# cwi-dis/cwipc_util

Hardware: AMD Instinct MI355X
Metric: Mpoints/s filtered (voxel downsample, 10M-pt synthetic) + achieved HBM GB/s (higher is better)
Workload: dtype f32 coordinates in, i64 fixed-point sums, u8 colours; 1 GPU; cwipc_synthetic(10000000) -> cwipc_downsample(+0.01) [BASELINE configs[1]]; points_per_gpu=9998244, bytes_per_gpu=159971904, outputs_per_gpu=39548, fused_points=39548, input_copies_rotated=4, inputs_resident_in_hbm=True

## Files before the change

### cwipc_util_amd/csrc/kernels_voxel.hip

```cpp
#include "internal.hpp"

#include <atomic>
#include <chrono>

#include <cstring>
#include <rocprim/device/device_radix_sort.hpp>

#include <cfloat>
#include <type_traits>
#include <cmath>

#include "voxel_anchor.hpp"
#include "voxel_common.hpp"

namespace cwipc_amd {

namespace {

#include "voxel_k1_general.inc"
#include "voxel_k1_fast.inc"
#include "voxel_partition.inc"
#include "voxel_finalize.inc"

struct PendingVoxel : DeferredResult {
    std::recursive_mutex lock;
    std::shared_ptr<DeviceSoA> src, spec_dst, result;
    volatile unsigned long long *words = nullptr;
    hipStream_t stream = nullptr;
    uint32_t seq = 0, spec_cap = 0;
    float cellsize = 0;
    bool known = false, ok = false, settled = false;
    uint32_t err = 0, m = 0;
    bool leaf_split = true;
    GridSpec gspec{0, 0u, 0u, 0ull};
    bool partitioned = false;
    uint32_t scatter = 0, steps_total = 0;
    uint32_t leaves = 0;
    bool outcome_locked();
    bool outcome() { std::lock_guard<std::recursive_mutex> g(lock); return outcome_locked(); }
    std::shared_ptr<DeviceSoA> settle() override;
};

std::atomic<size_t> g_workspace_bytes{0};
constexpr size_t GRID_BYTES = (size_t)CELLS * RECORD_WORDS * 8;
constexpr size_t HEAD_CTRL_BYTES = 256;

struct Workspace {
    int device = -1;
    size_t grid_bytes = 0;
    int cus = 0, cus_device = -1;
    uint32_t leaf_cap = 0;
    size_t list_cap = 0;
    size_t bbox_cap = 0;
    void *head = nullptr;
    size_t head_bytes = 0;
    int parity = 0;
    uint32_t seq = 0;
    uint32_t last_m = 0;
    uint32_t last_m_grid = 0;
    int shrink = 0;
    int calm = 0;
    bool incoherent = false;
    bool no_fast = false;
    int streak = 0;
    int roomy = 0;
    uint32_t shrink_to = 0;
    void note_leaves(uint32_t leaves) {
        uint32_t need = 4;
        while (need < leaves) need <<= 1;
        if (need * 4 <= leaf_cap) {
            if (++roomy >= 8) shrink_to = need;
        } else {
            roomy = 0;
            shrink_to = 0;
        }
    }
    uint32_t *host_words = nullptr;
    std::shared_ptr<struct PendingVoxel> pending;
    size_t hint_n = 0;
    float hint_cell = 0.f;
    bool hint_split = true;
    bool head_clean[2] = {false, false};
    unsigned long long *leaf_keys = nullptr;
    unsigned long long *hash_keys = nullptr;
    uint32_t *hash_ids = nullptr;
    unsigned long long *records = nullptr;
    uint32_t *occupied = nullptr;
    uint32_t *order = nullptr;
    uint32_t *gbits = nullptr;
    uint32_t *gprefix = nullptr, *gblock = nullptr;
    size_t gwords_cap = 0;
    float *bboxes = nullptr;
    float *part = nullptr;
    size_t part_stride = 0;
    uint32_t *part_hist = nullptr;
    size_t part_rows = 0;
    uint32_t *ctrl = nullptr;
    uint32_t *bitmaps = nullptr;
    uint32_t *seg_count = nullptr;
    float *faces = nullptr;
    uint32_t faces_host[FACE_TABLE_WORDS];
    double faces_mn0[3] = {0, 0, 0};
    double faces_res = 0;
    bool faces_valid = false;
    void drop_partition_buffers() {
        if (part) { (void)hipFree(part); g_workspace_bytes -= 16 * part_stride; }
        if (part_hist) (void)hipFree(part_hist);
        part = nullptr; part_hist = nullptr; part_stride = 0; part_rows = 0;
    }
    VoxWork work() const { return VoxWork{leaf_keys, records, occupied, ctrl, bboxes, faces, bitmaps, seg_count, hash_keys, hash_ids}; }
    char *bind_head(int blk) {
        char *h = (char *)head + (size_t)blk * head_bytes;
        ctrl = (uint32_t *)h;
        leaf_keys = (unsigned long long *)(h + HEAD_CTRL_BYTES);
        seg_count = (uint32_t *)(h + HEAD_CTRL_BYTES + (size_t)leaf_cap * 8);
        hash_keys = (unsigned long long *)(h + HEAD_CTRL_BYTES + (size_t)leaf_cap * 8 + (size_t)leaf_cap * RANK_SEGS * sizeof(uint32_t));
        hash_ids = (uint32_t *)((char *)hash_keys + (size_t)leaf_cap * 4 * 8);
        return h;
    }
    void free_grids() {
        if (head) (void)hipFree(head);
        if (records) (void)hipFree(records);
        if (bitmaps) (void)hipFree(bitmaps);
        head = nullptr; ctrl = nullptr; leaf_keys = nullptr; seg_count = nullptr; records = nullptr; bitmaps = nullptr;
        g_workspace_bytes -= grid_bytes;
        grid_bytes = 0;
        leaf_cap = 0;
    }
    void free_index_bitmap() {
        if (gbits) (void)hipFree(gbits);
        if (gprefix) (void)hipFree(gprefix);
        if (gblock) (void)hipFree(gblock);
        gbits = gprefix = gblock = nullptr; gwords_cap = 0;
    }
    void release() {
        free_grids();
        head_bytes = 0;
        if (occupied) (void)hipFree(occupied);
        if (order) (void)hipFree(order);
        free_index_bitmap();
        if (bboxes) (void)hipFree(bboxes);
        drop_partition_buffers();
        if (faces) (void)hipFree(faces);
        if (host_words) (void)hipHostFree(host_words);
        host_words = nullptr;
        occupied = nullptr; order = nullptr; bboxes = nullptr; faces = nullptr;
        list_cap = 0; bbox_cap = 0;
        faces_valid = false;
    }
    ~Workspace() { release(); }
};

std::mutex g_ws_pool_mutex;
std::vector<Workspace *> *g_ws_pool = new std::vector<Workspace *>();

constexpr int MAX_WS = 2 + ThreadCtx::EXTRA_STREAMS;
struct WorkspaceLease {
    Workspace *ws[MAX_WS] = {nullptr, nullptr, nullptr, nullptr};
    Workspace &get(int which) {
        if (!ws[which]) {
            const int dev = current_device();
            std::lock_guard<std::mutex> lock(g_ws_pool_mutex);
            for (size_t i = 0; i < g_ws_pool->size(); i++) {
                if ((*g_ws_pool)[i]->device == dev) {
                    ws[which] = (*g_ws_pool)[i];
                    g_ws_pool->erase(g_ws_pool->begin() + (long)i);
                    break;
                }
            }
            if (!ws[which]) ws[which] = new Workspace();
        }
        return *ws[which];
    }
    ~WorkspaceLease() {
        bool any = false;
        for (int i = 0; i < MAX_WS; i++) any = any || ws[i];
        if (any) (void)hipDeviceSynchronize();
        for (int i = 0; i < MAX_WS; i++)
            if (ws[i] && ws[i]->pending) (void)ws[i]->pending->outcome();
        std::vector<Workspace *> surplus;
        {
            std::lock_guard<std::mutex> lock(g_ws_pool_mutex);
            for (int i = 0; i < MAX_WS; i++) {
                if (!ws[i]) continue;
                if (g_ws_pool->size() < 8) g_ws_pool->push_back(ws[i]);
                else surplus.push_back(ws[i]);
            }
        }
        for (Workspace *w : surplus) delete w;
    }
};
thread_local WorkspaceLease t_ws;
thread_local int t_ws_next = 0;
thread_local uint32_t t_busy_sample = 0;
thread_local bool t_busy_sampled = false;
thread_local int t_ws_idle = 0;

hipStream_t &workspace_stream(ThreadCtx &c, int i) {
    if (i >= 2) (void)c.extra_stream(i - 2);
    return i == 0 ? c.stream : i == 1 ? c.stream_alt : c.stream_extra[i - 2];
}

struct StreamOfWorkspace {
    ThreadCtx &c;
    hipStream_t *other = nullptr;
    StreamOfWorkspace(ThreadCtx &ctx, int which) : c(ctx) {
        if (which > 0 && workspace_stream(c, which)) other = &workspace_stream(c, which);
        if (other) std::swap(c.stream, *other);
    }
    ~StreamOfWorkspace() {
        if (other) std::swap(c.stream, *other);
    }
};

bool ensure_workspace(Workspace &ws, size_t n, uint32_t leaf_cap, uint32_t nranges, hipStream_t s) {
    const int dev = current_device();
    if (ws.device != dev) {
        ws.release();
        const int lds = (int)sizeof(LdsTable);
        CW_HIP_TRY(hipFuncSetAttribute(reinterpret_cast<const void *>(&voxel_accumulate_kernel<0>), hipFuncAttributeMaxDynamicSharedMemorySize, lds));
        CW_HIP_TRY(hipFuncSetAttribute(reinterpret_cast<const void *>(&voxel_accumulate_kernel<1>), hipFuncAttributeMaxDynamicSharedMemorySize, lds));
        CW_HIP_TRY(hipFuncSetAttribute(reinterpret_cast<const void *>(&voxel_accumulate_kernel<2>), hipFuncAttributeMaxDynamicSharedMemorySize, lds));
        const int lds_fast = (int)sizeof(FastTable);
        CW_HIP_TRY(hipFuncSetAttribute(reinterpret_cast<const void *>(&voxel_accumulate_fast_kernel<0>), hipFuncAttributeMaxDynamicSharedMemorySize, lds_fast));
        CW_HIP_TRY(hipFuncSetAttribute(reinterpret_cast<const void *>(&voxel_accumulate_fast_kernel<1>), hipFuncAttributeMaxDynamicSharedMemorySize, lds_fast));
        CW_HIP_TRY(hipFuncSetAttribute(reinterpret_cast<const void *>(&partition_scatter_kernel), hipFuncAttributeMaxDynamicSharedMemorySize, (int)sizeof(PartLds)));
        ws.device = dev;
    }
    if (ws.leaf_cap < leaf_cap) {
        ws.free_grids();
        ws.head_bytes = HEAD_CTRL_BYTES + (size_t)leaf_cap * 8 + (size_t)leaf_cap * RANK_SEGS * sizeof(uint32_t) + (size_t)leaf_cap * 4 * (8 + 4);
        ws.head_bytes = (ws.head_bytes + 255) & ~(size_t)255;
        CW_HIP_TRY(hipMalloc(&ws.head, 2 * ws.head_bytes));
        ws.head_clean[0] = ws.head_clean[1] = false;
        ws.parity = 0;
        CW_HIP_TRY(hipMalloc((void **)&ws.bitmaps, (size_t)leaf_cap * BITWORDS * sizeof(uint32_t)));
        CW_HIP_TRY(hipMemsetAsync(ws.bitmaps, 0, (size_t)leaf_cap * BITWORDS * sizeof(uint32_t), s));
        CW_HIP_TRY(hipMalloc((void **)&ws.records, (size_t)leaf_cap * GRID_BYTES));
        CW_HIP_TRY(hipMemsetAsync(ws.records, 0, (size_t)leaf_cap * GRID_BYTES, s));
        ws.leaf_cap = leaf_cap;
        ws.grid_bytes = (size_t)leaf_cap * (GRID_BYTES + BITWORDS * sizeof(uint32_t)) + 2 * ws.head_bytes;
        g_workspace_bytes += ws.grid_bytes;
    }
    if (ws.list_cap < n) {
        if (ws.occupied) (void)hipFree(ws.occupied);
        if (ws.order) (void)hipFree(ws.order);
        ws.occupied = nullptr; ws.order = nullptr; ws.list_cap = 0;
        CW_HIP_TRY(hipMalloc((void **)&ws.occupied, n * sizeof(uint32_t)));
        CW_HIP_TRY(hipMalloc((void **)&ws.order, n * sizeof(uint32_t)));
        ws.list_cap = n;
    }
    if (ws.bbox_cap < nranges) {
        if (ws.bboxes) (void)hipFree(ws.bboxes);
        ws.bboxes = nullptr; ws.bbox_cap = 0;
        CW_HIP_TRY(hipMalloc((void **)&ws.bboxes, 2 * (size_t)nranges * 6 * sizeof(float)));
        ws.bbox_cap = nranges;
    }
    if (!ws.faces) CW_HIP_TRY(hipMalloc((void **)&ws.faces, FACE_TABLE_WORDS * sizeof(uint32_t)));
    if (!ws.host_words) {
        CW_HIP_TRY(hipHostMalloc((void **)&ws.host_words, 2 * C_WORDS * sizeof(uint32_t), hipHostMallocDefault));
        memset(ws.host_words, 0, 2 * C_WORDS * sizeof(uint32_t));
    }
    return true;
}

bool fetch_first_point(const DeviceSoA &src, ThreadCtx &c) {
    if (src.has_first) return true;
    float *h = (float *)c.host_words;
    hipLaunchKernelGGL(first_point_kernel, dim3(1), dim3(1), 0, c.stream, src.x(), src.y(), src.z(), h);
    bool ok = hipGetLastError() == hipSuccess;
    ok = c.sync() && ok;
    if (!ok) return hip_failed(hipGetLastError(), "fetch of the first point", __FILE__, __LINE__);
    src.first[0] = h[0]; src.first[1] = h[1]; src.first[2] = h[2];
    src.has_first = true;
    return true;
}

struct PassReport {
    uint32_t w[C_SEQ];
    bool seen = false;
    uint32_t operator[](int i) const { return w[i]; }
};

template <class StreamWait>
PassReport read_report(volatile unsigned long long *words, uint32_t seq, bool poll, const StreamWait &stream_wait) {
    PassReport r;
    const auto take = [&]() {
        for (int i = 0; i < C_SEQ; i++) {
            const unsigned long long w = words[i];
            if ((uint32_t)(w >> 32) != seq) return false;
            r.w[i] = (uint32_t)w;
        }
        return true;
    };
    if (poll) {
        const auto t_give_up = std::chrono::steady_clock::now() + std::chrono::microseconds(poll_budget_us());
        for (int spin = 0;; spin++) {
            if ((uint32_t)(words[C_COUNT] >> 32) == seq && take()) { r.seen = true; break; }
            if ((spin & 255) == 255 && std::chrono::steady_clock::now() > t_give_up) break;
            __builtin_ia32_pause();
        }
    }
    if (!r.seen && stream_wait()) r.seen = take();
    std::atomic_thread_fence(std::memory_order_acquire);
    return r;
}

bool grid_fits(const PassReport &hw, const GridSpec &spec) {
    const unsigned long long cells = (unsigned long long)hw[C_DIVB] * hw[C_DIVB + 1] * hw[C_DIVB + 2];
    return hw[C_COUNT] <= spec.m_cap && cells <= spec.cells_max && (cells + 31) / 32 <= spec.words_cap;
}

std::shared_ptr<DeviceSoA> empty_result(bool leaf_split) {
    if (leaf_split) return soa_alloc(0);
    cwipc_log(CWIPC_LOG_LEVEL_ERROR, "cwipc_downsample", "VoxelGrid filter produced empty pointcloud");
    return nullptr;
}

void learn_from_pass(Workspace &ws, bool leaf_split, bool went_through, uint32_t m, bool partitioned, uint32_t scatter, size_t steps_total) {
    (leaf_split ? ws.last_m : ws.last_m_grid) = went_through ? m : 0;
    if (partitioned && (size_t)scatter * 4 < steps_total) ws.incoherent = false;
}

bool PendingVoxel::outcome_locked() {
    if (known) return ok;
    const PassReport hw = read_report(words, seq, true, [&]() {
        if (hipStreamSynchronize(stream) != hipSuccess) (void)hipGetLastError();
        return true;
    });
    known = true;
    err = hw.seen ? hw[C_ERR] : 0x80000000u;
    m = hw.seen ? hw[C_COUNT] : 0u;
    scatter = hw.seen ? hw[C_SCATTER] : 0xffffffffu;
    leaves = hw.seen ? hw[C_LEAVES] : 0u;
    ok = hw.seen && err == 0u && m <= spec_cap;
    if (ok && !leaf_split) ok = grid_fits(hw, gspec);
    return ok;
}

std::shared_ptr<DeviceSoA> PendingVoxel::settle() {
    std::lock_guard<std::recursive_mutex> g(lock);
    if (settled) return result;
    if (outcome_locked()) {
        if (m == 0) {
            result = empty_result(leaf_split);
        } else {
            spec_dst->npoints = m;
            result = spec_dst;
        }
    } else {
        int code = 0;
        result = voxel_downsample(src, cellsize, leaf_split, &code, nullptr);
    }
    spec_dst.reset();
    src.reset();
    settled = true;
    return result;
}

struct VoxCall {
    ThreadCtx &c;
    Workspace &ws;
    const std::shared_ptr<DeviceSoA> &src_ptr;
    const DeviceSoA &src;
    const float cellsize;
    const bool leaf_split;
    const size_t n;
    int cus = 0;
    size_t steps_total = 0, nwaves = 0, part_nseg = 0;
    uint32_t nblocks = 0, faces_host[FACE_TABLE_WORDS];
    double faces_key_mn0[3] = {0, 0, 0};
    bool partition = false;
    VoxParams P;
    uint32_t leaf_cap = 0;
    int mode;
    bool local_leaves = true;
    bool ok = true, used_fast = false;
    hipError_t launch_err = hipSuccess;
    uint32_t seq = 0, err = 0, spec_cap = 0;
    VoxWork W;
    char *next_head = nullptr;
    FastPlan fplan{0u, 0u, 0u, 0u};
    std::shared_ptr<DeviceSoA> spec_dst;
    GridSpec gspec{0, 0u, 0u, 0ull};
    unsigned long long bitmap_max = GRID_BITMAP_MAX_CELLS;
    VoxCall(ThreadCtx &ctx, Workspace &w, const std::shared_ptr<DeviceSoA> &s, float cell, bool split)
        : c(ctx), ws(w), src_ptr(s), src(*s), cellsize(cell), leaf_split(split), n(s->npoints), mode(split ? 1 : 0) {}

    bool collect_pending(); void plan(); bool anchor_and_faces(std::shared_ptr<DeviceSoA> &early); bool partition_buffers(); bool first_leaf_cap();
    bool setup_pass(); void launch_accumulate(); void launch_replay(); void launch_speculative();
    void launch_grid_finalize(const GridSpec &spec, uint32_t count, uint32_t words, DeviceSoA &dst);
    bool hand_out(int attempt, std::shared_ptr<DeferredResult> *deferred); PassReport await_report(); void adapt_workgroups(const PassReport &hw);
    std::shared_ptr<DeviceSoA> finalize(const PassReport &hw, uint32_t m);
    bool retry_or_report(int attempt, const PassReport &hw, uint32_t m, std::shared_ptr<DeviceSoA> &dst);
};

int pick_workspace(ThreadCtx &c) {
    static const int max_ws = []() { const char *e = getenv("CWIPC_WORKSPACES"); const int v = e ? atoi(e) : 3; return v < 1 ? 1 : v > MAX_WS ? MAX_WS : v; }();
    int have = 0;
    while (have < MAX_WS && t_ws.ws[have]) have++;
    const bool sampled = t_busy_sampled;
    t_busy_sampled = false;
    const auto busy = [&](int i) {
        if (sampled) return ((t_busy_sample >> i) & 1u) != 0u;
        hipStream_t s = workspace_stream(c, i);
        const bool b = s && hipStreamQuery(s) == hipErrorNotReady;
        (void)hipGetLastError();
        return b;
    };
    int which = 0;
    if (have > 0) {
        which = t_ws_next % have;
        if (have < max_ws && busy(which)) {
            which = have;
        } else if (have > 1 && !t_ws.ws[have - 1]->pending) {
            bool idle = true;
            for (int i = 0; i < have && idle; i++) idle = !busy(i);
            t_ws_idle = idle ? t_ws_idle + 1 : 0;
            if (t_ws_idle >= 16) {
                delete t_ws.ws[have - 1];
                t_ws.ws[have - 1] = nullptr;
                have--;
                t_ws_idle = 0;
                which = which % have;
            }
        }
    }
    t_ws_next = which + 1;
    return which;
}

bool VoxCall::collect_pending() {
    if (!ws.pending) return true;
    const std::shared_ptr<PendingVoxel> p = ws.pending;
    ws.pending.reset();
    const bool went_through = p->outcome();
    learn_from_pass(ws, p->leaf_split, went_through, p->m, went_through && p->partitioned, p->scatter, p->steps_total);
    if (went_through) {
        ws.note_leaves(p->leaves);
        return true;
    }
    ws.streak = 0;
    if (p->err & (ERR_FAST_PATH | ERR_CELL_RANGE)) ws.no_fast = true;
    CW_LAUNCH("clean_by_bitmap", clean_by_bitmap_kernel, dim3(ws.leaf_cap * RANK_SEGS), dim3(RANK_THREADS), 0, c.stream, ws.work());
    if (!c.sync()) { hip_failed(hipGetLastError(), "voxel workspace clean-up", __FILE__, __LINE__); return false; }
    return true;
}

void VoxCall::plan() {
    if (ws.cus_device != current_device() || ws.cus <= 0) {
        int cus_now = 0;
        if (hipDeviceGetAttribute(&cus_now, hipDeviceAttributeMultiprocessorCount, current_device()) != hipSuccess || cus_now <= 0) cus_now = 256;
        ws.cus = cus_now;
        ws.cus_device = current_device();
    }
    static const int spare_knob = []() { const char *e = getenv("CWIPC_SPARE_CUS"); return e ? atoi(e) : -1; }();
    const int spare_cus = spare_knob >= 0 ? spare_knob : ws.cus / 32;
    cus = ws.cus - spare_cus > 8 ? ws.cus - spare_cus : ws.cus;
    if (ws.hint_cell != cellsize || ws.hint_split != leaf_split || n > 2 * ws.hint_n || 2 * n < ws.hint_n) {
        ws.shrink = 0;
        ws.calm = 0;
        ws.incoherent = false;
        ws.no_fast = false;
        ws.streak = 0;
    }
    ws.hint_cell = cellsize;
    ws.hint_split = leaf_split;
    ws.hint_n = n;
    steps_total = (n + WAVE_STEP - 1) / WAVE_STEP;
    nwaves = general_plan_waves(n, cus, ws.shrink);
    nblocks = (uint32_t)(nwaves / K1_WAVES);

    memset(&P, 0, sizeof(P));
    P.n = n;
    P.per_wave = general_plan_per_wave(n, nwaves);
    P.nranges = (uint32_t)nwaves;
    P.leaf = cellsize;
    P.inv_leaf = 1.0f / cellsize;
    P.vox_unit = 1.0 / (double)P.inv_leaf;
    P.q_unit = P.vox_unit / 8388608.0;
    P.leaf_d = (double)cellsize;
    const float octree_cellsize = (8 * 8) * cellsize;
    P.res = (double)octree_cellsize;
    P.leaf_split = leaf_split ? 1 : 0;
#ifdef CWIPC_DEBUG_KNOBS
    static const uint32_t ablate_knob = []() { const char *e = getenv("CWIPC_VOXEL_ABLATE"); return e ? (uint32_t)atoi(e) : 0u; }();
    if (ablate_knob) cwipc_log(CWIPC_LOG_LEVEL_WARNING, "cwipc_downsample", "CWIPC_VOXEL_ABLATE is set: results are WRONG (timing experiments only)");
    P.ablate = ablate_knob;
#endif
}

bool VoxCall::anchor_and_faces(std::shared_ptr<DeviceSoA> &early) {
    memset(faces_host, 0, sizeof(faces_host));
    if (leaf_split) {
        if (!fetch_first_point(src, c)) return false;
        float anchor[3] = {src.first[0], src.first[1], src.first[2]};
        if (!(std::isfinite(anchor[0]) && std::isfinite(anchor[1]) && std::isfinite(anchor[2]))) {
            float *h = (float *)c.host_words;
            hipLaunchKernelGGL(first_finite_kernel, dim3(1), dim3(1024), 0, c.stream, src.x(), src.y(), src.z(), n, h);
            bool ok = hipGetLastError() == hipSuccess;
            ok = c.sync() && ok;
            if (!ok) { hip_failed(hipGetLastError(), "search for the first finite point", __FILE__, __LINE__); return false; }
            if (h[3] == 0.0f) { early = soa_alloc(0); return false; }
            anchor[0] = h[0]; anchor[1] = h[1]; anchor[2] = h[2];
        }
        const double pp[3] = {(double)anchor[0], (double)anchor[1], (double)anchor[2]};
        first_box(pp, P.res, P.mn0, P.mx0, P.depth0);
        for (int a = 0; a < 3; a++) {
            P.ib[a] = (int)floor(P.mn0[a] / P.leaf_d);
            P.face_base[a] = 1 - FACE_BACK;
        }
        const bool cached = ws.faces_valid && ws.faces_res == P.res && ws.faces_mn0[0] == P.mn0[0] && ws.faces_mn0[1] == P.mn0[1] && ws.faces_mn0[2] == P.mn0[2];
        if (cached) {
            memcpy(faces_host, ws.faces_host, sizeof(faces_host));
        } else {
            fill_face_table(P.mn0, P.res, P.face_base, P.inv_leaf, faces_host);
        }
        faces_key_mn0[0] = P.mn0[0]; faces_key_mn0[1] = P.mn0[1]; faces_key_mn0[2] = P.mn0[2];
    } else {
        for (int a = 0; a < 3; a++) P.ib[a] = 2;
    }
    return true;
}

bool VoxCall::partition_buffers() {
    static const bool partition_off = []() { const char *e = getenv("CWIPC_VOXEL_PARTITION"); return e && atoi(e) == 0; }();
    partition = ws.incoherent && !partition_off && n >= 65536;
    const size_t part_stride = (n + 1023) & ~(size_t)1023;
    part_nseg = (nblocks + PART_SEG_ROWS - 1) / PART_SEG_ROWS;
    if (partition) {
        if (ws.part_stride < part_stride || ws.part_rows < nblocks) {
            ws.drop_partition_buffers();
            if (hipMalloc((void **)&ws.part, 16 * part_stride) != hipSuccess ||
                hipMalloc((void **)&ws.part_hist, ((size_t)nblocks + part_nseg + 1) * PART_BUCKETS * sizeof(uint32_t)) != hipSuccess) {
                (void)hipGetLastError();
                ws.drop_partition_buffers();
                hip_failed(hipErrorOutOfMemory, "voxel partition buffers", __FILE__, __LINE__);
                return false;
            }
            ws.part_stride = part_stride;
            ws.part_rows = nblocks;
            g_workspace_bytes += 16 * part_stride;
        }
    } else if (ws.part) {
        ws.drop_partition_buffers();
    }
    return true;
}

bool VoxCall::first_leaf_cap() {
    if (ws.shrink_to && ws.shrink_to < ws.leaf_cap) {
        if (!c.sync()) return false;
        ws.free_grids();
    }
    leaf_cap = ws.leaf_cap ? ws.leaf_cap : (ws.shrink_to ? ws.shrink_to : 4);
    if (ws.shrink_to) ws.roomy = 0;
    ws.shrink_to = 0;
    return true;
}

bool VoxCall::setup_pass() {
    if (!ensure_workspace(ws, n, leaf_cap, (uint32_t)nwaves, c.stream)) return false;
    P.leaf_mask = 4 * ws.leaf_cap - 1;
    P.list_cap = (uint32_t)(ws.list_cap > 0xffffffffu ? 0xffffffffu : ws.list_cap);
    seq = ++ws.seq ? ws.seq : ++ws.seq;
    for (int i = 0; i < C_SEQ; i++) ws.host_words[2 * i + 1] = 0;
    const int blk = ws.parity;
    char *head = ws.bind_head(blk);
    next_head = (char *)ws.head + (size_t)(1 - blk) * ws.head_bytes;
    W = ws.work();
    ok = true;
    if (!ws.head_clean[blk]) ok = hipMemsetAsync(head, 0, ws.head_bytes, c.stream) == hipSuccess;
    ws.head_clean[blk] = false;
    if (ok && mode == 1 && !(ws.faces_valid && memcmp(ws.faces_host, faces_host, sizeof(faces_host)) == 0)) {
        uint32_t *stage = (uint32_t *)c.staging(sizeof(faces_host));
        ok = stage != nullptr;
        if (ok) {
            memcpy(stage, faces_host, sizeof(faces_host));
            ok = hipMemcpyAsync(ws.faces, stage, sizeof(faces_host), hipMemcpyHostToDevice, c.stream) == hipSuccess;
            memcpy(ws.faces_host, faces_host, sizeof(faces_host));
            ws.faces_valid = ok;
            ws.faces_res = P.res;
            ws.faces_mn0[0] = faces_key_mn0[0]; ws.faces_mn0[1] = faces_key_mn0[1]; ws.faces_mn0[2] = faces_key_mn0[2];
        }
    }
    if (!ok) { hip_failed(hipGetLastError(), "voxel workspace setup", __FILE__, __LINE__); return false; }
    return true;
}

K1Params k1_params(const VoxParams &P, bool local_leaves) {
    K1Params K;
    memset(&K, 0, sizeof(K));
    K.n = (uint32_t)P.n; K.per_wave = (uint32_t)P.per_wave;
    K.inv_leaf = P.inv_leaf;
    K.ib0 = P.ib[0]; K.ib1 = P.ib[1]; K.ib2 = P.ib[2];
    K.fb0 = P.face_base[0]; K.fb1 = P.face_base[1]; K.fb2 = P.face_base[2];
    K.leaf_mask = P.leaf_mask; K.list_cap = P.list_cap; K.ablate = P.ablate;
    K.local_leaves = local_leaves ? 1u : 0u;
    K.want_list = P.leaf_split ? 0u : 1u;
    K.mn0[0] = P.mn0[0]; K.mn0[1] = P.mn0[1]; K.mn0[2] = P.mn0[2];
    K.res = P.res;
    return K;
}

FastParams fast_params(const K1Params &K, const FastPlan &plan) {
    FastParams F;
    memset(&F, 0, sizeof(F));
    F.n = K.n; F.per_wg = plan.per_wg; F.inv_leaf = K.inv_leaf;
    F.range_base_q = plan.base_q; F.range_inc_q = plan.inc_q;
    F.ib0 = K.ib0; F.ib1 = K.ib1; F.ib2 = K.ib2;
    F.fb0 = K.fb0; F.fb1 = K.fb1; F.fb2 = K.fb2;
    F.leaf_mask = K.leaf_mask; F.list_cap = K.list_cap; F.want_list = K.want_list;
    return F;
}

void VoxCall::launch_accumulate() {
    const K1Params K = k1_params(P, local_leaves);
    static const bool fast_off = []() { const char *e = getenv("CWIPC_VOXEL_GENERAL"); return e && atoi(e) != 0; }();
    const bool fast = mode != 2 && !ws.no_fast && ws.shrink == 0 && !fast_off && !partition;
    const float *kx = src.x(), *ky = src.y(), *kz = src.z();
    const uint32_t *kw = src.rgbt();
    VoxWork Wk = W;
    if (partition) {
        float *px = ws.part, *py = px + ws.part_stride, *pz = py + ws.part_stride;
        uint32_t *pw = (uint32_t *)(pz + ws.part_stride);
        const uint32_t padded = (uint32_t)((n + WAVE_STEP - 1) / WAVE_STEP * WAVE_STEP);
        uint32_t *rows = ws.part_hist, *seg = rows + ws.part_rows * PART_BUCKETS, *start = seg + part_nseg * PART_BUCKETS;
        const uint32_t per_wg = (uint32_t)(P.per_wave * K1_WAVES);
        CW_LAUNCH("partition_count", partition_count_kernel, dim3(nblocks), dim3(K1_THREADS), 0, c.stream, (uint32_t)n, per_wg, P.inv_leaf,
                  src.x(), src.y(), src.z(), ws.bboxes, rows, ws.ctrl);
        CW_LAUNCH("partition_scan", partition_segsum_kernel, dim3((unsigned)part_nseg, PART_BUCKETS / 256), dim3(256), 0, c.stream, rows, nblocks, seg);
        CW_LAUNCH("partition_scan", partition_starts_kernel, dim3(1), dim3(K1_THREADS), 0, c.stream, seg, (uint32_t)part_nseg, start);
        CW_LAUNCH("partition_scatter", partition_scatter_kernel, dim3(nblocks), dim3(K1_THREADS), sizeof(PartLds), c.stream,
                  (uint32_t)n, per_wg, padded, P.inv_leaf, src.x(), src.y(), src.z(), src.rgbt(), px, py, pz, pw, rows, seg, start);
        kx = px; ky = py; kz = pz; kw = pw;
        Wk.bboxes = ws.bboxes + (size_t)ws.bbox_cap * 6;
    }
    used_fast = fast;
    fplan = FastPlan{0u, 0u, 0u, 0u};
    if (fast) {
        static const int stagger_knob = []() { const char *e = getenv("CWIPC_K1_STAGGER"); return e ? atoi(e) : 25; }();
        fplan = fast_plan(n, cus, stagger_knob);
        FastParams F = fast_params(K, fplan);
#ifdef CWIPC_DEBUG_KNOBS
        static const uint32_t fast_dbg = []() { const char *e = getenv("CWIPC_FAST_DBG"); return e ? (uint32_t)atoi(e) : 0u; }();
        if (fast_dbg) cwipc_log(CWIPC_LOG_LEVEL_WARNING, "cwipc_downsample", "CWIPC_FAST_DBG is set: results are WRONG (timing experiments only)");
        F.dbg = fast_dbg;
#endif
        if (mode == 0) {
            CW_LAUNCH("voxel_accumulate", voxel_accumulate_fast_kernel<0>, dim3(fplan.blocks), dim3(K1_THREADS), sizeof(FastTable), c.stream, F, src.x(),
                      src.y(), src.z(), src.rgbt(), W);
        } else {
            CW_LAUNCH("voxel_accumulate", voxel_accumulate_fast_kernel<1>, dim3(fplan.blocks), dim3(K1_THREADS), sizeof(FastTable), c.stream, F, src.x(),
                      src.y(), src.z(), src.rgbt(), W);
        }
    } else if (mode == 0) {
        CW_LAUNCH("voxel_accumulate_general", voxel_accumulate_kernel<0>, dim3(nblocks), dim3(K1_THREADS), sizeof(LdsTable), c.stream, K, kx, ky, kz, kw, Wk);
    } else if (mode == 1) {
        CW_LAUNCH("voxel_accumulate_general", voxel_accumulate_kernel<1>, dim3(nblocks), dim3(K1_THREADS), sizeof(LdsTable), c.stream, K, kx, ky, kz, kw, Wk);
    } else {
        CW_LAUNCH("voxel_accumulate_exact", voxel_accumulate_kernel<2>, dim3(nblocks), dim3(K1_THREADS), sizeof(LdsTable), c.stream, K, kx, ky, kz, kw, Wk);
    }
}

void VoxCall::launch_replay() {
    VoxParams Pr = P;
    if (used_fast) {
        Pr.per_wave = fplan.per_wg;
        Pr.nranges = fplan.blocks;
        Pr.range_base_q = fplan.base_q; Pr.range_inc_q = fplan.inc_q;
    } else if (partition) {
        Pr.per_wave = P.per_wave * K1_WAVES;
        Pr.nranges = nblocks;
    }
    CW_LAUNCH("octree_replay", octree_replay_kernel, dim3(1), dim3(1024), 0, c.stream, Pr, src.x(), src.y(), src.z(), ws.bboxes, ws.ctrl,
              ws.leaf_keys, ws.leaf_cap, (uint32_t *)next_head, (uint32_t)(ws.head_bytes / 4), ws.host_words, seq);
    launch_err = hipGetLastError();
    ok = launch_err == hipSuccess;
    const int blk = ws.parity;
    ws.head_clean[1 - blk] = ok;
    ws.parity = 1 - blk;
}

void VoxCall::launch_grid_finalize(const GridSpec &spec, uint32_t count, uint32_t words, DeviceSoA &dst) {
    const bool prof = !spec.on;
#define GRID_LAUNCH(name, ...) do { if (prof) CW_LAUNCH(name, __VA_ARGS__); else hipLaunchKernelGGL(__VA_ARGS__); } while (0)
    const uint32_t m_host = spec.on ? 0u : count, nwords_host = spec.on ? 0u : words;
    const unsigned mgrid = (count + 255) / 256, nblk = (unsigned)((words + GB_WORDS_PER_BLOCK - 1) / GB_WORDS_PER_BLOCK);
    GRID_LAUNCH("grid_mark", grid_mark_kernel, dim3(mgrid), dim3(256), 0, c.stream, P, W, m_host, spec, ws.gbits, ws.order);
    GRID_LAUNCH("grid_block", grid_block_kernel, dim3(nblk), dim3(256), 0, c.stream, W, spec, ws.gbits, nwords_host, ws.gprefix, ws.gblock);
    GRID_LAUNCH("grid_blockscan", grid_blockscan_kernel, dim3(1), dim3(1024), 0, c.stream, W, spec, ws.gblock, nwords_host);
    GRID_LAUNCH("grid_emit", grid_emit_kernel, dim3(mgrid), dim3(256), 0, c.stream, P, W, m_host, spec, ws.order, ws.gbits, ws.gprefix, ws.gblock,
                dst.x(), dst.y(), dst.z(), dst.rgbt());
    GRID_LAUNCH("grid_unmark", grid_unmark_kernel, dim3(mgrid), dim3(256), 0, c.stream, W, m_host, spec, ws.order, ws.gbits);
#undef GRID_LAUNCH
}

void VoxCall::launch_speculative() {
    spec_dst.reset();
    spec_cap = 0;
    if (ok && leaf_split && ws.last_m > 0 && !profiling_enabled()) {
        spec_cap = ws.last_m + ws.last_m / 4 + 1024;
        spec_dst = soa_alloc(spec_cap);
        if (spec_dst) {
            hipLaunchKernelGGL(rank_emit_kernel, dim3(ws.leaf_cap * RANK_SEGS), dim3(RANK_THREADS), 0, c.stream, P, W, ws.leaf_cap, spec_cap, 1, ws.order,
                               spec_dst->x(), spec_dst->y(), spec_dst->z(), spec_dst->rgbt());
            spec_dst->mark_pending(c.stream);
        }
    }
    gspec = GridSpec{0, 0u, 0u, 0ull};
    bitmap_max = GRID_BITMAP_MAX_CELLS;
    if (const char *e = getenv("CWIPC_GRID_BITMAP_MAX")) bitmap_max = strtoull(e, nullptr, 10);
    if (ok && !leaf_split && ws.last_m_grid > 0 && ws.gwords_cap > 0 && !profiling_enabled()) {
        spec_cap = ws.last_m_grid + ws.last_m_grid / 4 + 1024;
        if (spec_cap > P.list_cap) spec_cap = P.list_cap;
        spec_dst = soa_alloc(spec_cap);
        if (spec_dst) {
            gspec = GridSpec{1, spec_cap, (uint32_t)std::min<size_t>(ws.gwords_cap, 0xffffffffu), bitmap_max};
            launch_grid_finalize(gspec, spec_cap, gspec.words_cap, *spec_dst);
            spec_dst->mark_pending(c.stream);
        }
    }
}

bool VoxCall::hand_out(int attempt, std::shared_ptr<DeferredResult> *deferred) {
    static const bool defer_on = []() { const char *e = getenv("CWIPC_DEFER"); return !e || atoi(e) != 0; }();
    if (!(deferred && defer_on && attempt == 0 && ok && spec_dst && (leaf_split || gspec.on) && ws.streak >= 2)) return false;
    auto p = std::make_shared<PendingVoxel>();
    p->src = src_ptr;
    p->spec_dst = spec_dst;
    p->words = reinterpret_cast<volatile unsigned long long *>(ws.host_words);
    p->stream = c.stream;
    p->seq = seq;
    p->spec_cap = spec_cap;
    p->cellsize = cellsize;
    p->leaf_split = leaf_split;
    p->gspec = gspec;
    p->partitioned = partition;
    p->steps_total = (uint32_t)steps_total;
    src.note_reader(c.stream);
    ws.pending = p;
    *deferred = p;
    return true;
}

PassReport VoxCall::await_report() {
    volatile unsigned long long *words = reinterpret_cast<volatile unsigned long long *>(ws.host_words);
    const PassReport hw = read_report(words, seq, ok && !profiling_enabled(), [&]() { ok = c.sync() && ok; return ok; });
    if (ok && !hw.seen) { ok = false; cwipc_log(CWIPC_LOG_LEVEL_ERROR, "cwipc_downsample", "voxel grid failed: the replay kernel did not report"); }
    return hw;
}

#ifdef CWIPC_DEBUG_KNOBS
void log_fast_stamps(uint32_t fast_blocks) {
    unsigned long long st[2][16];
    (void)hipDeviceSynchronize();
    if (hipMemcpyFromSymbol(st, HIP_SYMBOL(g_fast_stamps), sizeof(st)) == hipSuccess) {
        for (int w = 0; w < 2; w++) {
            std::string line = "debug: workgroup " + std::string(w ? "mid" : "0") + " phases (us since its start): ";
            const char *names[9] = {"start", "table ready", "steps done", "boxes out", "entries compacted", "keys decoded", "leaf ids", "records updated", "end"};
            for (int i = 1; i < 9; i++) line += std::string(names[i]) + " " + std::to_string((double)(st[w][i] - st[w][0]) * 0.01).substr(0, 5) + "; ";
            cwipc_log(CWIPC_LOG_LEVEL_WARNING, "cwipc_downsample", line);
        }
        static unsigned long long wt[1024][4];
        if (hipMemcpyFromSymbol(wt, HIP_SYMBOL(g_wg_times), sizeof(wt)) == hipSuccess && fast_blocks > 0 && fast_blocks <= 1024) {
            unsigned long long t0 = ~0ull, s_max = 0, e_min = ~0ull, e_max = 0, d_min = ~0ull, d_max = 0, a_max = 0;
            for (uint32_t b = 0; b < fast_blocks; b++) {
                t0 = std::min(t0, wt[b][0]); s_max = std::max(s_max, wt[b][0]);
                e_min = std::min(e_min, wt[b][3]); e_max = std::max(e_max, wt[b][3]);
                d_min = std::min(d_min, wt[b][3] - wt[b][0]); d_max = std::max(d_max, wt[b][3] - wt[b][0]);
                a_max = std::max(a_max, wt[b][2]);
            }
            char buf[256];
            snprintf(buf, sizeof(buf), "debug: %u workgroups: last start %.2f us after the first; records updated between %.2f and %.2f us; all waves done by %.2f; a workgroup lives %.2f to %.2f us",
                     fast_blocks, (double)(s_max - t0) * 0.01, (double)(e_min - t0) * 0.01, (double)(e_max - t0) * 0.01, (double)(a_max - t0) * 0.01, (double)d_min * 0.01, (double)d_max * 0.01);
            cwipc_log(CWIPC_LOG_LEVEL_WARNING, "cwipc_downsample", buf);
            if (const char *path = getenv("CWIPC_FAST_STAMPS_FILE")) {
                if (FILE *f = fopen(path, "w")) {
                    fprintf(f, "# workgroup start stream_done(thread 0's wave) all_waves_done end   (us since the first start)\n");
                    for (uint32_t b = 0; b < fast_blocks; b++)
                        fprintf(f, "%u %.2f %.2f %.2f %.2f\n", b, (double)(wt[b][0] - t0) * 0.01, (double)(wt[b][1] - t0) * 0.01, (double)(wt[b][2] - t0) * 0.01, (double)(wt[b][3] - t0) * 0.01);
                    fclose(f);
                }
            }
        }
        unsigned long long wd[K1_WAVES];
        if (hipMemcpyFromSymbol(wd, HIP_SYMBOL(g_fast_wave_done), sizeof(wd)) == hipSuccess) {
            std::string line = "debug: workgroup 0, waves done with their steps at (us):";
            for (int w = 0; w < K1_WAVES; w++) line += " " + std::to_string((double)(wd[w] - st[0][0]) * 0.01).substr(0, 5);
            cwipc_log(CWIPC_LOG_LEVEL_WARNING, "cwipc_downsample", line);
        }
    }
}
#endif

void VoxCall::adapt_workgroups(const PassReport &hw) {
    const uint32_t fallbacks = hw[C_FALLBACK], maxload = hw[C_MAXLOAD];
    if (!used_fast && !err && n >= 65536 && 2 * ((size_t)hw[C_FLUSHED] + fallbacks) > n && n > 4 * (size_t)hw[C_COUNT]) {
        ws.incoherent = true;
        ws.shrink = 0;
        ws.calm = 0;
    } else if (ws.incoherent) {
    } else if (ws.shrink >= 2 && (size_t)fallbacks * 2 > n) {
        ws.incoherent = true;
        ws.shrink = 0;
        ws.calm = 0;
    } else if ((size_t)fallbacks * 64 > n && ws.shrink < 6) {
        ws.shrink++;
        ws.calm = 0;
    } else if (ws.shrink > 0 && fallbacks == 0 && maxload * 3 < (uint32_t)LTAB) {
        if (++ws.calm >= 4) { ws.shrink--; ws.calm = 0; }
    } else {
        ws.calm = 0;
    }
}

std::shared_ptr<DeviceSoA> VoxCall::finalize(const PassReport &hw, uint32_t m) {
    std::shared_ptr<DeviceSoA> dst;
    unsigned long long *keys_in = nullptr, *keys_out = nullptr;
    uint32_t *vals_in = nullptr, *vals_out = nullptr;
    void *sort_tmp = nullptr;
    const unsigned mgrid = (m + 255) / 256;

    bool ranked = false;
    bool grid_ranked = false;
    if (!err && m && !leaf_split && spec_dst && gspec.on && grid_fits(hw, gspec)) {
        dst = spec_dst;
        dst->npoints = m;
        grid_ranked = true;
    }
    if (!err && m && leaf_split && spec_dst && m <= spec_cap) {
        dst = spec_dst;
        dst->npoints = m;
        ranked = true;
    }
    spec_dst.reset();
    if (!ranked && !err && m && leaf_split) {
        dst = soa_alloc(m);
        if (!dst) {
            err |= 0x80000000u;
        } else {
            CW_LAUNCH("rank_emit", rank_emit_kernel, dim3(ws.leaf_cap * RANK_SEGS), dim3(RANK_THREADS), 0, c.stream, P, W, ws.leaf_cap, m, 0, ws.order,
                      dst->x(), dst->y(), dst->z(), dst->rgbt());
            dst->mark_pending(c.stream);
            ranked = true;
        }
    }
    if (!err && m && !leaf_split && !grid_ranked) {
        const unsigned long long cells = (unsigned long long)hw[C_DIVB] * hw[C_DIVB + 1] * hw[C_DIVB + 2];
        if (cells <= bitmap_max) {
            const uint32_t nwords = (uint32_t)((cells + 31) / 32);
            bool ready = true;
            if (ws.gwords_cap < nwords) {
                ws.free_index_bitmap();
                const size_t cap = std::max<size_t>((size_t)nwords * 2, (size_t)1 << 16);
                ready = hipMalloc((void **)&ws.gbits, cap * 4) == hipSuccess && hipMalloc((void **)&ws.gprefix, cap * 4) == hipSuccess &&
                        hipMalloc((void **)&ws.gblock, (cap / GB_WORDS_PER_BLOCK + 2) * 4) == hipSuccess &&
                        hipMemsetAsync(ws.gbits, 0, cap * 4, c.stream) == hipSuccess;
                if (ready) ws.gwords_cap = cap; else (void)hipGetLastError();
            }
            dst = ready ? soa_alloc(m) : nullptr;
            if (dst) {
                launch_grid_finalize(GridSpec{0, 0u, 0u, 0ull}, m, nwords, *dst);
                dst->mark_pending(c.stream);
                grid_ranked = true;
            }
        }
    }
    if (!err && m && !leaf_split && !grid_ranked) {
        dst = soa_alloc(m);
        keys_in = (unsigned long long *)pool_alloc((size_t)m * 8 * 2);
        vals_in = (uint32_t *)pool_alloc((size_t)m * 4 * 2);
        if (!dst || !keys_in || !vals_in) {
            err |= 0x80000000u;
        } else {
            keys_out = keys_in + m;
            vals_out = vals_in + m;
            CW_LAUNCH("make_sort_keys", make_sort_keys_kernel, dim3(mgrid), dim3(256), 0, c.stream, P, W, m, keys_in, vals_in);
            const unsigned end_bit = 32;
            size_t tmp_bytes = 0;
            hipError_t e = rocprim::radix_sort_pairs(nullptr, tmp_bytes, keys_in, keys_out, vals_in, vals_out, (size_t)m, 0u, end_bit, c.stream);
            if (e == hipSuccess) {
                sort_tmp = pool_alloc(tmp_bytes ? tmp_bytes : 256);
                if (!sort_tmp) e = hipErrorOutOfMemory;
            }
            if (e == hipSuccess) {
                if (profiling_enabled()) profile_begin("radix_sort_pairs", c.stream);
                e = rocprim::radix_sort_pairs(sort_tmp, tmp_bytes, keys_in, keys_out, vals_in, vals_out, (size_t)m, 0u, end_bit, c.stream);
                if (profiling_enabled()) profile_end(c.stream);
            }
            if (e != hipSuccess) {
                hip_failed(e, "rocprim::radix_sort_pairs", __FILE__, __LINE__);
                err |= 0x80000000u;
            }
        }
    }
    if (leaf_split && !ranked) {
        CW_LAUNCH("clean_by_bitmap", clean_by_bitmap_kernel, dim3(ws.leaf_cap * RANK_SEGS), dim3(RANK_THREADS), 0, c.stream, W);
        ok = c.sync() && ok;
    }
    if (!leaf_split && m && !grid_ranked) {
        const int emit = (!err && dst) ? 1 : 0;
        CW_LAUNCH("emit_and_clean", emit_and_clean_kernel, dim3(mgrid), dim3(256), 0, c.stream, P, W, m, vals_out, emit ? dst->x() : nullptr,
                  emit ? dst->y() : nullptr, emit ? dst->z() : nullptr, emit ? dst->rgbt() : nullptr, emit);
        if (emit) ok = hipMemcpyAsync(c.host_words, ws.ctrl, sizeof(uint32_t), hipMemcpyDeviceToHost, c.stream) == hipSuccess;
        ok = c.sync() && ok;
        if (emit && ok) err |= c.host_words[C_ERR];
    }
    pool_free(keys_in);
    pool_free(vals_in);
    pool_free(sort_tmp);
    return dst;
}

bool VoxCall::retry_or_report(int attempt, const PassReport &hw, uint32_t m, std::shared_ptr<DeviceSoA> &dst) {
    const uint32_t retryable = ERR_LEAVES | ERR_FACE_TABLE | ERR_LOCAL_LEAVES | ERR_LIST_FULL | ERR_FAST_PATH | (used_fast ? ERR_CELL_RANGE : 0u);
    if (used_fast && (err & (ERR_FAST_PATH | ERR_CELL_RANGE)) && !(err & ~retryable)) {
        ws.no_fast = true;
        return true;
    }
    if ((err & (ERR_LEAVES | ERR_FACE_TABLE | ERR_LOCAL_LEAVES)) && !(err & ~retryable)) {
        if (err & ERR_LOCAL_LEAVES) local_leaves = false;
        if (err & ERR_FACE_TABLE) mode = 2;
        if (err & ERR_LEAVES) {
            if ((size_t)leaf_cap * 4 * GRID_BYTES > ((size_t)200 << 30)) {
                cwipc_log(CWIPC_LOG_LEVEL_ERROR, "cwipc_downsample", "voxel grid failed: the cloud spans more octree leaves than fit in device memory");
                dst = nullptr;
                return false;
            }
            leaf_cap *= 4;
        }
        return true;
    }
    if (err) {
        std::string why;
        if (err & ERR_GRID_OVERFLOW) why += " VoxelGrid: leaf size is too small for the input dataset, integer indices would overflow;";
        if (err & ERR_RANGE) why += " voxel or leaf index out of range;";
        if (err & (ERR_DEPTH | ERR_LEAF_RANGE)) why += " octree deeper than 14 levels;";
        if (err & ERR_CELL_RANGE) why += " voxel outside its leaf grid;";
        if (err & ERR_LIST_FULL) why += " occupied list full;";
        if (err & 0x80000000u) why += " device allocation or sort failure;";
        cwipc_log(CWIPC_LOG_LEVEL_ERROR, "cwipc_downsample", "voxel grid failed:" + why);
        dst = nullptr;
        return false;
    }
    if (!m) {
        dst = empty_result(leaf_split);
        return false;
    }
    ws.streak = attempt == 0 ? ws.streak + 1 : 0;
    ws.note_leaves(hw[C_LEAVES]);
    return false;
}

}

void voxel_sample_streams() {
    ThreadCtx &c = tctx();
    if (!c.ensure()) return;
    uint32_t bits = 0;
    for (int i = 0; i < MAX_WS && t_ws.ws[i]; i++) {
        hipStream_t s = workspace_stream(c, i);
        if (s && hipStreamQuery(s) == hipErrorNotReady) bits |= 1u << i;
        (void)hipGetLastError();
    }
    t_busy_sample = bits;
    t_busy_sampled = true;
}

std::shared_ptr<DeviceSoA> voxel_downsample(const std::shared_ptr<DeviceSoA> &src_ptr, float cellsize, bool leaf_split, int *error_code,
                                            std::shared_ptr<DeferredResult> *deferred) {
    ThreadCtx &c = tctx();
    if (!c.ensure()) return nullptr;
    const int which = pick_workspace(c);
    Workspace &ws = t_ws.get(which);
    StreamOfWorkspace on_its_stream(c, which);
    VoxCall k(c, ws, src_ptr, cellsize, leaf_split);
    if (!k.collect_pending()) return nullptr;
    k.src.wait_on(c.stream);
    if (k.n >= ((size_t)1 << 31)) {
        cwipc_log(CWIPC_LOG_LEVEL_ERROR, "cwipc_downsample", "voxel grid failed: more than 2^31 points");
        return nullptr;
    }
    k.plan();
    std::shared_ptr<DeviceSoA> result;
    if (!k.anchor_and_faces(result)) return result;
    if (!k.partition_buffers() || !k.first_leaf_cap()) return nullptr;
    for (int attempt = 0; attempt < 10; attempt++) {
        if (!k.setup_pass()) return nullptr;
        k.launch_accumulate();
        k.launch_replay();
        k.launch_speculative();
        if (k.hand_out(attempt, deferred)) return nullptr;
        const PassReport hw = k.await_report();
        if (!k.ok) { hip_failed(k.launch_err != hipSuccess ? k.launch_err : hipGetLastError(), "voxel_accumulate", __FILE__, __LINE__); return nullptr; }
        k.err = hw[C_ERR];
#ifdef CWIPC_DEBUG_KNOBS
        if (k.used_fast && getenv("CWIPC_FAST_STAMPS")) log_fast_stamps(k.fplan.blocks);
#endif
        const uint32_t m = hw[C_COUNT] < k.P.list_cap ? hw[C_COUNT] : k.P.list_cap;
        learn_from_pass(ws, leaf_split, !k.err, m, k.partition, hw[C_SCATTER], k.steps_total);
        if (!k.partition) k.adapt_workgroups(hw);
        result = k.finalize(hw, m);
        if (error_code) *error_code = (int)k.err;
        if (!k.ok) { hip_failed(hipGetLastError(), "voxel emit", __FILE__, __LINE__); return nullptr; }
        if (!k.retry_or_report(attempt, hw, m, result)) return result;
    }
    cwipc_log(CWIPC_LOG_LEVEL_ERROR, "cwipc_downsample", "voxel grid failed: could not size the workspace");
    return nullptr;
}

size_t voxel_workspace_bytes() { return g_workspace_bytes.load(); }

size_t voxel_release_pooled_workspaces() {
    std::vector<Workspace *> gone;
    {
        std::lock_guard<std::mutex> lock(g_ws_pool_mutex);
        gone.swap(*g_ws_pool);
    }
    if (!gone.empty()) (void)hipDeviceSynchronize();
    for (Workspace *w : gone) {
        if (w->pending) (void)w->pending->outcome();
        delete w;
    }
    return gone.size();
}

}

extern "C" _CWIPC_UTIL_EXPORT size_t cwipc_hip_workspace_bytes(void) { return cwipc_amd::voxel_workspace_bytes(); }
extern "C" _CWIPC_UTIL_EXPORT size_t cwipc_hip_workspace_trim(void) { return cwipc_amd::voxel_release_pooled_workspaces(); }
```

### cwipc_util_amd/csrc/voxel_anchor.hpp

```cpp
#pragma once
#include <algorithm>
#include <cfloat>
#include <cmath>
#include <cstring>
#include "voxel_common.hpp"
namespace cwipc_amd {
namespace {

void first_box(const double p[3], double res, double mn[3], double mx[3], int &depth) {
    const double eps = (double)FLT_EPSILON;
    unsigned max_key = 0;
    for (int a = 0; a < 3; a++) {
        mn[a] = p[a] - res / 2;
        mx[a] = p[a] + res / 2;
        unsigned mk = (unsigned)ceil((mx[a] - mn[a] - eps) / res);
        max_key = mk > max_key ? mk : max_key;
    }
    unsigned max_voxels = max_key > 2 ? max_key : 2;
    double d = ceil(log2((double)max_voxels) - eps);
    d = d > 32 ? 32 : (d < 0 ? 0 : d);
    depth = (int)d;
    double side = (double)(1u << depth) * res;
    for (int a = 0; a < 3; a++) {
        double oversize = (side - (mx[a] - mn[a])) / 2.0;
        if (oversize > eps) {
            mn[a] -= oversize;
            mx[a] += oversize;
        }
    }
}

template <class Pred>
float first_float_where(const Pred &passes, float guess) {
    const auto to_ord = [](float f) { int32_t b; memcpy(&b, &f, 4); return b >= 0 ? (int64_t)b : -(int64_t)(b & 0x7fffffff); };
    const auto from_ord = [](int64_t o) { int32_t b = o >= 0 ? (int32_t)o : (int32_t)(0x80000000u | (uint32_t)(-o)); float f; memcpy(&f, &b, 4); return f; };
    const int64_t lowest = to_ord(-FLT_MAX), highest = to_ord(FLT_MAX);
    if (!(guess >= -FLT_MAX && guess <= FLT_MAX)) guess = 0.f;
    int64_t lo, hi;
    const int64_t g = to_ord(guess);
    if (passes(from_ord(g))) {
        hi = g;
        int64_t step = 1;
        for (;;) {
            lo = hi - step;
            if (lo <= lowest) { lo = lowest; if (passes(from_ord(lo))) return -FLT_MAX; break; }
            if (!passes(from_ord(lo))) break;
            hi = lo;
            step *= 2;
        }
    } else {
        lo = g;
        int64_t step = 1;
        for (;;) {
            hi = lo + step;
            if (hi >= highest) { hi = highest; if (!passes(from_ord(hi))) return INFINITY; break; }
            if (passes(from_ord(hi))) break;
            lo = hi;
            step *= 2;
        }
    }
    while (hi - lo > 1) {
        const int64_t mid = lo + (hi - lo) / 2;
        if (passes(from_ord(mid))) hi = mid; else lo = mid;
    }
    return from_ord(hi);
}

float leaf_threshold(double mn0, double res, int m) {
    const double md = (double)m;
    return first_float_where([&](float p) { return floor(((double)p - mn0) / res) >= md; }, (float)(mn0 + md * res));
}

float voxel_upper_bound(float inv_leaf, int voxel) {
    return first_float_where([&](float p) { return floorf(p * inv_leaf) > (float)voxel; }, (float)(((double)voxel + 1.0) / (double)inv_leaf));
}

void fill_face_table(const double mn0[3], double res, const int face_base[3], float inv_leaf, uint32_t faces_host[FACE_TABLE_WORDS]) {
    for (int a = 0; a < 3; a++) {
        for (int i = 0; i < FACES; i++) {
            const float T = leaf_threshold(mn0[a], res, face_base[a] + i);
            const float g = floorf(T * inv_leaf);
            const bool sane = std::isfinite(T) && fabsf(g) < 1.0e9f;
            const int tf = sane ? (int)g : (T > 0 ? INT32_MAX : INT32_MIN);
            const float Tv = sane ? voxel_upper_bound(inv_leaf, tf) : T;
            memcpy(&faces_host[FT_T + a * FACES + i], &T, 4);
            memcpy(&faces_host[FT_TV + a * FACES + i], &Tv, 4);
            memcpy(&faces_host[FT_TF + a * FACES + i], &tf, 4);
        }
    }
}

inline size_t general_plan_waves(size_t n, int cus, int shrink) {
    size_t nwaves = ((size_t)cus * K1_WAVES) << shrink;
    const size_t steps_total = (n + WAVE_STEP - 1) / WAVE_STEP;
    if (nwaves > steps_total) nwaves = ((steps_total + K1_WAVES - 1) / K1_WAVES) * K1_WAVES;
    const size_t min_waves = (n + MAX_POINTS_PER_WAVE - 1) / MAX_POINTS_PER_WAVE;
    if (nwaves < min_waves) nwaves = ((min_waves + K1_WAVES - 1) / K1_WAVES) * K1_WAVES;
    return nwaves;
}
inline size_t general_plan_per_wave(size_t n, size_t nwaves) { return (((n + nwaves - 1) / nwaves + WAVE_STEP - 1) / WAVE_STEP) * WAVE_STEP; }

struct FastPlan { uint32_t blocks, per_wg, base_q, inc_q; };
inline FastPlan fast_plan(size_t n, int cus, int stagger_knob) {
    const size_t steps_total = (n + WAVE_STEP - 1) / WAVE_STEP;
    const size_t wg_steps = std::min<size_t>(std::max<size_t>((steps_total + cus - 1) / cus, 1), MAX_POINTS_PER_WAVE * K1_WAVES / WAVE_STEP);
    FastPlan plan{(uint32_t)((steps_total + wg_steps - 1) / wg_steps), (uint32_t)(wg_steps * WAVE_STEP), 0u, 0u};
    const uint32_t fast_blocks = plan.blocks;
    if (stagger_knob > 0 && stagger_knob < 60 && fast_blocks >= 64 && steps_total >= (size_t)24 * fast_blocks && n < ((size_t)1 << 31)) {
        const double mean_q = (double)steps_total * 1024.0 / (double)fast_blocks, s_frac = stagger_knob / 100.0;
        const size_t max_steps = MAX_POINTS_PER_WAVE * K1_WAVES / WAVE_STEP;
        uint32_t inc = (uint32_t)ceil(2.0 * s_frac * mean_q / (double)(fast_blocks - 1));
        uint32_t base = (uint32_t)ceil(mean_q * (1.0 - s_frac));
        while (range_first_step(fast_blocks, base, inc) < steps_total) base++;
        const size_t longest = (size_t)((base + (unsigned long long)(fast_blocks - 1) * inc + 2047) >> 10);
        if (base >= 1024 && longest <= max_steps) {
            plan.base_q = base; plan.inc_q = inc;
            plan.per_wg = (uint32_t)(longest * WAVE_STEP);
        }
    }
    return plan;
}

}
}
```

### cwipc_util_amd/csrc/voxel_common.hpp

```cpp
#pragma once
#include <cstddef>
#include <cstdint>
#if defined(__HIPCC__) || defined(__CUDACC__)
#define CWIPC_HOST_DEVICE __host__ __device__
#else
#define CWIPC_HOST_DEVICE
#endif
namespace cwipc_amd {
namespace {

constexpr int K1_THREADS = 1024;
constexpr int K1_WAVES = K1_THREADS / 64;
constexpr int WAVE_STEP = 256;
constexpr size_t MAX_POINTS_PER_WAVE = 3840;
constexpr int LTAB = 2048;
constexpr int LTAB_PROBES = 32;
constexpr int GRID_DIM = 68;
constexpr int CELLS = GRID_DIM * GRID_DIM * GRID_DIM;
constexpr int CELL_BITS = 19;
constexpr int BITWORDS = CELLS / 32;
constexpr uint32_t KEY_EMPTY = 0xffffffffu;
constexpr int HIST = 256;
constexpr int LOCAL_LEAVES = 64;
constexpr int RANK_THREADS = 256;
constexpr int RANK_SEGS = 16;
constexpr int SEG_WORDS = (BITWORDS + RANK_SEGS - 1) / RANK_SEGS;
constexpr int WORDS_PER_THREAD = (SEG_WORDS + RANK_THREADS - 1) / RANK_THREADS;
constexpr int RECORD_WORDS = 8;
constexpr int FACES = 128;
constexpr int FACE_BACK = 63;
constexpr int FT_T = 0, FT_TV = 3 * FACES, FT_TF = 6 * FACES, FACE_TABLE_WORDS = 9 * FACES;

enum : uint32_t {
    ERR_RANGE = 1,
    ERR_LEAVES = 2,
    ERR_DEPTH = 4,
    ERR_GRID_OVERFLOW = 8,
    ERR_LEAF_RANGE = 16,
    ERR_FACE_TABLE = 32,
    ERR_CELL_RANGE = 64,
    ERR_LIST_FULL = 128,
    ERR_LOCAL_LEAVES = 512,
    ERR_FAST_PATH = 1024,
};

enum {
    C_ERR = 0, C_COUNT = 1, C_DEPTH = 2, C_EVENTS = 3, C_SHIFT = 4 , C_MINB = 10, C_DIVB = 13,
    C_FALLBACK = 16,
    C_MAXLOAD = 17,
    C_SCATTER = 18,
    C_FLUSHED = 19,
    C_LEAVES = 20,
    C_SEQ = 31,
    C_WORDS = 32
};

struct VoxParams {
    size_t n;
    size_t per_wave;
    uint32_t range_base_q, range_inc_q;
    uint32_t nranges;
    float inv_leaf;
    float leaf;
    double leaf_d;
    double vox_unit;
    double q_unit;
    double res;
    double mn0[3], mx0[3];
    int depth0;
    int ib[3];
    int face_base[3];
    int leaf_split;
    uint32_t leaf_mask;
    uint32_t list_cap;
    uint32_t ablate;
};

struct VoxWork {
    unsigned long long *leaf_keys;
    unsigned long long *records;
    uint32_t *occupied;
    uint32_t *ctrl;
    float *bboxes;
    const float *faces;
    uint32_t *bitmaps;
    uint32_t *seg_count;
    unsigned long long *hash_keys;
    uint32_t *hash_ids;
};

inline CWIPC_HOST_DEVICE uint32_t range_first_step(uint32_t b, uint32_t base_q, uint32_t inc_q) {
    const unsigned long long bb = b;
    return (uint32_t)((bb * base_q + (unsigned long long)inc_q * (bb * (bb > 0 ? bb - 1 : 0) / 2)) >> 10);
}

inline CWIPC_HOST_DEVICE uint64_t mix64(uint64_t k) {
    k ^= k >> 33; k *= 0xff51afd7ed558ccdull;
    k ^= k >> 33; k *= 0xc4ceb9fe1a85ec53ull;
    k ^= k >> 33;
    return k;
}

#if defined(__HIPCC__)
__device__ __forceinline__ unsigned long long pack_leaf(int lx, int ly, int lz) {
    return (1ull << 63) | ((unsigned long long)(uint32_t)(lx & 0x1fffff)) | ((unsigned long long)(uint32_t)(ly & 0x1fffff) << 21) |
           ((unsigned long long)(uint32_t)(lz & 0x1fffff) << 42);
}
__device__ __forceinline__ int unpack_leaf(unsigned long long v, int axis) {
    int t = (int)((v >> (21 * axis)) & 0x1fffff);
    return (t << 11) >> 11;
}

__device__ __forceinline__ uint32_t leaf_lookup(const VoxWork &W, uint32_t mask, unsigned long long k) {
    const uint32_t cap = (mask + 1u) >> 2;
    uint32_t pos = (uint32_t)mix64(k) & mask;
    uint32_t probes = 0;
    for (uint32_t guard = 0; guard < (1u << 22); guard++) {
        unsigned long long cur = __hip_atomic_load(&W.hash_keys[pos], __ATOMIC_RELAXED, __HIP_MEMORY_SCOPE_AGENT);
        if (cur == 0ull) {
            cur = atomicCAS(&W.hash_keys[pos], 0ull, k);
            if (cur == 0ull) {
                const uint32_t id = atomicAdd(&W.ctrl[C_LEAVES], 1u);
                if (id < cap) {
                    W.leaf_keys[id] = k;
                    __hip_atomic_store(&W.hash_ids[pos], id + 1u, __ATOMIC_RELAXED, __HIP_MEMORY_SCOPE_AGENT);
                    return id;
                }
                atomicOr(&W.ctrl[C_ERR], ERR_LEAVES);
                __hip_atomic_store(&W.hash_ids[pos], 0xffffffffu, __ATOMIC_RELAXED, __HIP_MEMORY_SCOPE_AGENT);
                return 0xffffffffu;
            }
        }
        if (cur == k) {
            const uint32_t v = __hip_atomic_load(&W.hash_ids[pos], __ATOMIC_RELAXED, __HIP_MEMORY_SCOPE_AGENT);
            if (v != 0u) return v == 0xffffffffu ? 0xffffffffu : v - 1u;
            continue;
        }
        pos = (pos + 1) & mask;
        if (++probes > mask) break;
    }
    atomicOr(&W.ctrl[C_ERR], ERR_LEAVES);
    return 0xffffffffu;
}

__device__ __forceinline__ uint32_t leaf_lookup_cached(const VoxWork &W, uint32_t mask, unsigned long long k) {
    uint32_t pos = (uint32_t)mix64(k) & mask;
    for (uint32_t probes = 0; probes < 8u; probes++) {
        const unsigned long long cur = __hip_atomic_load(&W.hash_keys[pos], __ATOMIC_RELAXED, __HIP_MEMORY_SCOPE_WAVEFRONT);
        if (cur == k) {
            const uint32_t v = __hip_atomic_load(&W.hash_ids[pos], __ATOMIC_RELAXED, __HIP_MEMORY_SCOPE_WAVEFRONT);
            if (v != 0u && v != 0xffffffffu) return v - 1u;
            break;
        }
        if (cur == 0ull) break;
        pos = (pos + 1) & mask;
    }
    return leaf_lookup(W, mask, k);
}

__device__ __forceinline__ unsigned long long *record_ptr(const VoxWork &W, uint32_t key) {
    return W.records + ((size_t)(key >> CELL_BITS) * CELLS + (key & ((1u << CELL_BITS) - 1))) * RECORD_WORDS;
}

__device__ __forceinline__ uint32_t slice_of(uint32_t key) {
    const uint32_t cell = key & ((1u << CELL_BITS) - 1);
    return (key >> CELL_BITS) * RANK_SEGS + (cell >> 5) / SEG_WORDS;
}

__device__ __forceinline__ void mark_occupied(const VoxWork &W, uint32_t key) {
    const uint32_t cell = key & ((1u << CELL_BITS) - 1);
    atomicOr(&W.bitmaps[(size_t)(key >> CELL_BITS) * BITWORDS + (cell >> 5)], 1u << (cell & 31u));
}

constexpr uint32_t Q_ONE_BITS = 0x3f800000u;
__device__ __forceinline__ float voxel_fract(float prod) { return __builtin_amdgcn_fractf(prod); }
__device__ __forceinline__ uint32_t voxel_offset(float prod) { return __float_as_uint(__fadd_rn(voxel_fract(prod), 1.0f)) - Q_ONE_BITS; }
#endif
}
}
```

### cwipc_util_amd/csrc/voxel_k1_fast.inc

```

#ifdef CWIPC_DEBUG_KNOBS
__device__ unsigned long long g_fast_stamps[2][16];
__device__ unsigned long long g_fast_wave_done[K1_WAVES];
__device__ unsigned long long g_wg_times[1024][4];
#define FAST_STAMP(i) do { if (threadIdx.x == 0) { const unsigned long long t_ = wall_clock64(); if (blockIdx.x == 0 || blockIdx.x == gridDim.x / 2) g_fast_stamps[blockIdx.x ? 1 : 0][i] = t_; \
    if (blockIdx.x < 1024 && ((i) == 0 || (i) == 2 || (i) == 3 || (i) == 7)) g_wg_times[blockIdx.x][(i) == 0 ? 0 : (i) == 2 ? 1 : (i) == 3 ? 2 : 3] = t_; } } while (0)
#else
#define FAST_STAMP(i) do { } while (0)
#endif

constexpr int KEY_SPAN_X = 1024, KEY_SPAN_Y = 1024, KEY_SPAN_Z = 4096;
constexpr unsigned long long KEY64_EMPTY = ~0ull;
constexpr uint32_t Q_NEG_ONE_BITS = 0u - Q_ONE_BITS;

typedef float f32x2 __attribute__((ext_vector_type(2)));

struct FastParams {
    uint32_t n, per_wg;
    uint32_t range_base_q, range_inc_q;
    float inv_leaf;
    int ib0, ib1, ib2;
    int fb0, fb1, fb2;
    uint32_t leaf_mask, list_cap, want_list;
    uint32_t dbg;
};

struct FastTable {
    unsigned long long key[LTAB];
    uint32_t tile[LTAB];
    unsigned long long a[LTAB];
    unsigned long long b[LTAB];
    unsigned long long c[LTAB];
    unsigned long long d[LTAB];
    uint32_t faces[FACE_TABLE_WORDS];
    uint32_t htag[HIST], hcnt[HIST];
    unsigned long long leaf_tab[LOCAL_LEAVES];
    uint32_t leaf_gid[LOCAL_LEAVES];
    alignas(16) float slab[K1_WAVES][12];
    int slab_j[K1_WAVES][4];
    int tmin[3], tmax[3];
    uint32_t nfresh, fresh_base, nused, err;
    uint32_t next_step;
    float wbox[K1_WAVES][6];
    alignas(16) uint32_t used[LTAB];
    uint32_t rec[LTAB];
    uint32_t fresh[LTAB];
};

__device__ __forceinline__ uint32_t linear_key(int ix, int iy, int iz) {
    uint32_t t, k;
    asm("v_lshl_add_u32 %0, %1, 10, %2" : "=v"(t) : "v"(iz), "v"(iy));
    asm("v_lshl_add_u32 %0, %1, 10, %2" : "=v"(k) : "v"(t), "v"(ix));
    return k;
}
__device__ __forceinline__ float min2f(float a, float b) {
    float r;
    asm("v_min_f32 %0, %1, %2" : "=v"(r) : "v"(a), "v"(b));
    return r;
}
__device__ __forceinline__ float max2f(float a, float b) {
    float r;
    asm("v_max_f32 %0, %1, %2" : "=v"(r) : "v"(a), "v"(b));
    return r;
}

__device__ __forceinline__ int cvt_floor_i32(float v) {
    int r;
    asm("v_cvt_flr_i32_f32 %0, %1" : "=v"(r) : "v"(v));
    return r;
}

__device__ __forceinline__ uint32_t fast_hash(uint32_t key, uint32_t side) {
    static_assert(LTAB <= 2048 && (LTAB & (LTAB - 1)) == 0, "11 bits at most");
    const uint32_t t = key ^ (key >> 13) ^ (side << 7);
    return (__umul24(t, 0x9E3779u) >> 13) & (uint32_t)(LTAB - 1);
}

__device__ __forceinline__ unsigned long long fast_find_begin(FastTable &L, uint32_t key, uint32_t side, bool active, uint32_t &slot) {
    slot = fast_hash(key, side);
    unsigned long long old = KEY64_EMPTY;
    if (active) old = atomicCAS(&L.key[slot], KEY64_EMPTY, u64_of(key, side));
    return old;
}
__device__ __forceinline__ bool fast_find_end(FastTable &L, uint32_t key, uint32_t side, bool active, unsigned long long old, uint32_t &slot, uint32_t &err) {
    const unsigned long long key64 = u64_of(key, side);
    bool pending = active && !(old == KEY64_EMPTY || old == key64);
#pragma unroll 1
    for (int probe = 1; probe < LTAB_PROBES; probe++) {
        if (__ballot(pending) == 0ull) break;
        if (pending) {
            slot = (slot + 1) & (LTAB - 1);
            old = atomicCAS(&L.key[slot], KEY64_EMPTY, key64);
            if (old == KEY64_EMPTY || old == key64) pending = false;
        }
    }
    if (__ballot(active && pending) != 0ull) err |= ERR_FAST_PATH;
    return active && !pending;
}
__device__ __forceinline__ bool fast_find(FastTable &L, uint32_t key, uint32_t side, bool active, uint32_t &slot, uint32_t &err) {
    const unsigned long long old = fast_find_begin(L, key, side, active, slot);
    return fast_find_end(L, key, side, active, old, slot, err);
}

__device__ __forceinline__ void fast_add_rest(FastTable &L, uint32_t slot, bool ok, uint32_t qz, uint32_t cr, uint32_t gb, uint32_t tile) {
    if (ok) {
        atomicAdd(&L.c[slot], u64_of(qz, (gb & 0xffffu) << 8));
        atomicAdd(&L.d[slot], u64_of(__builtin_amdgcn_alignbit(cr, cr, 16), (gb >> 16) << 8));
        if ((L.tile[slot] & tile) != tile) atomicOr(&L.tile[slot], tile);
    }
}

__device__ __forceinline__ uint32_t fast_leaf_slot(FastTable &L, unsigned long long k) {
    uint32_t pos = (((uint32_t)k ^ (uint32_t)(k >> 21) ^ (uint32_t)(k >> 42)) * 0x9E3779B1u) >> 26;
    for (int probe = 0; probe < LOCAL_LEAVES; probe++) {
        unsigned long long cur = L.leaf_tab[pos];
        if (cur == 0ull) {
            cur = atomicCAS(&L.leaf_tab[pos], 0ull, k);
            if (cur == 0ull) cur = k;
        }
        if (cur == k) return pos;
        pos = (pos + 1) & (LOCAL_LEAVES - 1);
    }
    return 0xffffffffu;
}

__device__ __forceinline__ uint32_t wave_inclusive_scan(uint32_t v) {
    v += (uint32_t)__builtin_amdgcn_update_dpp(0, (int)v, 0x111, 0xf, 0xf, true);
    v += (uint32_t)__builtin_amdgcn_update_dpp(0, (int)v, 0x112, 0xf, 0xf, true);
    v += (uint32_t)__builtin_amdgcn_update_dpp(0, (int)v, 0x114, 0xf, 0xf, true);
    v += (uint32_t)__builtin_amdgcn_update_dpp(0, (int)v, 0x118, 0xf, 0xf, true);
    v += (uint32_t)__builtin_amdgcn_update_dpp(0, (int)v, 0x142, 0xa, 0xf, false);
    v += (uint32_t)__builtin_amdgcn_update_dpp(0, (int)v, 0x143, 0xc, 0xf, false);
    return v;
}

__device__ __attribute__((noinline)) bool fast_refit(FastTable *Lp, int wave, float mn0, float mn1, float mn2, float mx0, float mx1, float mx2, float inv,
                                                      int ib0, int ib1, int ib2, int fb0, int fb1, int fb2) {
    FastTable &L = *Lp;
    float lo[3] = {mn0, mn1, mn2}, hi[3] = {mx0, mx1, mx2};
    for (int sft = 32; sft > 0; sft >>= 1) {
#pragma unroll
        for (int a = 0; a < 3; a++) {
            lo[a] = fminf(lo[a], __shfl_xor(lo[a], sft, 64));
            hi[a] = fmaxf(hi[a], __shfl_xor(hi[a], sft, 64));
        }
    }
    if (!(lo[0] <= hi[0])) return true;
    const int ib[3] = {ib0, ib1, ib2}, fb[3] = {fb0, fb1, fb2};
    bool bad = false;
#pragma unroll 1
    for (int a = 0; a < 3; a++) {
        const float *T = reinterpret_cast<const float *>(&L.faces[FT_T + a * FACES]);
        const float *TV = reinterpret_cast<const float *>(&L.faces[FT_TV + a * FACES]);
        const float lowest = lo[a], highest = hi[a];
        int i = L.slab_j[wave][a];
        if (i < 0) i = ((cvt_floor_i32(lowest * inv) - ib[a]) >> 6) - fb[a];
        i = max(0, min(i, FACES - 3));
        for (int it = 0; it < FACES && i > 0 && lowest < TV[i]; it++) i--;
        for (int it = 0; it < FACES && i < FACES - 3 && lowest >= TV[i + 1]; it++) i++;
        const float tlo = TV[i], tmid = T[i + 1], tv = TV[i + 1], thi = T[i + 2];
        if (!(lowest >= tlo && lowest < tv && highest < thi)) bad = true;
        if ((threadIdx.x & 63) == 0) {
            L.slab[wave][4 * a + 0] = tlo; L.slab[wave][4 * a + 1] = tmid; L.slab[wave][4 * a + 2] = tv; L.slab[wave][4 * a + 3] = thi;
            L.slab_j[wave][a] = i;
        }
    }
    return !bad;
}

template <int MODE>
__device__ __attribute__((noinline)) void fast_scout(FastTable *Lp, float inv_leaf, int ib0, int ib1, int ib2, int fb0, int fb1, int fb2, uint32_t leaf_mask,
                                                      unsigned long long *hash_keys, uint32_t *hash_ids, unsigned long long *leaf_keys, uint32_t *ctrl,
                                                      float f0, float f1, float f2) {
    FastTable &L = *Lp;
    const float f[3] = {f0, f1, f2};
    if (!__builtin_isfinite(f0 + f1 + f2)) return;
    const int ib[3] = {ib0, ib1, ib2}, fb[3] = {fb0, fb1, fb2};
    int l[3];
#pragma unroll
    for (int a = 0; a < 3; a++) {
        const int t = cvt_floor_i32(__fmul_rn(f[a], inv_leaf)) - ib[a];
        if (MODE == 0) {
            l[a] = t >> 6;
        } else {
            const int m = (t + 32) >> 6;
            const unsigned i = (unsigned)(m - fb[a]);
            if (!(i + 1u < (unsigned)FACES)) return;
            const float *T = reinterpret_cast<const float *>(&L.faces[FT_T + a * FACES]);
            l[a] = m - 1 + (f[a] >= T[i] ? 1 : 0) + (f[a] >= T[i + 1] ? 1 : 0);
        }
        if (!(l[a] > -(1 << 20) && l[a] < (1 << 20))) return;
    }
    const unsigned long long k = pack_leaf(l[0], l[1], l[2]);
    const uint32_t ls = fast_leaf_slot(L, k);
    if (ls == 0xffffffffu) return;
    VoxWork w{};
    w.hash_keys = hash_keys; w.hash_ids = hash_ids; w.leaf_keys = leaf_keys; w.ctrl = ctrl;
    L.leaf_gid[ls] = leaf_lookup(w, leaf_mask, k);
}

__device__ __forceinline__ void wave_box_to_63(float &n0, float &n1, float &n2, float &x0, float &x1, float &x2) {
#define CWIPC_BOX_STAGE(CTRL)                                \
    "v_min_f32_dpp %0, %0, %0 " CTRL "\n"                    \
    "v_min_f32_dpp %1, %1, %1 " CTRL "\n"                    \
    "v_min_f32_dpp %2, %2, %2 " CTRL "\n"                    \
    "v_max_f32_dpp %3, %3, %3 " CTRL "\n"                    \
    "v_max_f32_dpp %4, %4, %4 " CTRL "\n"                    \
    "v_max_f32_dpp %5, %5, %5 " CTRL "\n"
    asm volatile("s_nop 1\n"
                 CWIPC_BOX_STAGE("row_shr:1 row_mask:0xf bank_mask:0xf")
                 CWIPC_BOX_STAGE("row_shr:2 row_mask:0xf bank_mask:0xf")
                 CWIPC_BOX_STAGE("row_shr:4 row_mask:0xf bank_mask:0xf")
                 CWIPC_BOX_STAGE("row_shr:8 row_mask:0xf bank_mask:0xf")
                 CWIPC_BOX_STAGE("row_bcast:15 row_mask:0xa bank_mask:0xf")
                 CWIPC_BOX_STAGE("row_bcast:31 row_mask:0xc bank_mask:0xf")
                 : "+v"(n0), "+v"(n1), "+v"(n2), "+v"(x0), "+v"(x1), "+v"(x2));
#undef CWIPC_BOX_STAGE
}

__device__ __forceinline__ int fast_finish_head(FastTable &L, const FastParams &P, const VoxWork &W, uint32_t err, float bn0, float bn1, float bn2, float bx0, float bx1,
                                                float bx2, int &tmn0, int &tmn1, int &tmn2) {
    const int lane = threadIdx.x & 63, wave = threadIdx.x >> 6;
    const float inv = P.inv_leaf;
    if (__ballot(err != 0u) != 0ull) {
        for (int s = 32; s > 0; s >>= 1) err |= (uint32_t)__shfl_xor((int)err, s, 64);
        if (lane == 0) atomicOr(&L.err, err);
    }
    {
        float vlo0 = bn0, vlo1 = bn1, vlo2 = bn2, vhi0 = bx0, vhi1 = bx1, vhi2 = bx2;
        wave_box_to_63(vlo0, vlo1, vlo2, vhi0, vhi1, vhi2);
        if (lane == 63) {
            L.wbox[wave][0] = vlo0; L.wbox[wave][1] = vlo1; L.wbox[wave][2] = vlo2;
            L.wbox[wave][3] = vhi0; L.wbox[wave][4] = vhi1; L.wbox[wave][5] = vhi2;
            if (vlo0 <= vhi0) {
                atomicMin(&L.tmin[0], cvt_floor_i32(vlo0 * inv)); atomicMin(&L.tmin[1], cvt_floor_i32(vlo1 * inv)); atomicMin(&L.tmin[2], cvt_floor_i32(vlo2 * inv));
                atomicMax(&L.tmax[0], cvt_floor_i32(vhi0 * inv)); atomicMax(&L.tmax[1], cvt_floor_i32(vhi1 * inv)); atomicMax(&L.tmax[2], cvt_floor_i32(vhi2 * inv));
            }
        }
    }
    tmn0 = tmn1 = tmn2 = 0;
#ifdef CWIPC_DEBUG_KNOBS
    if (P.dbg & 8u) return 0;
#endif
    __syncthreads();
    FAST_STAMP(3);
    if (threadIdx.x < 6) {
        float v = L.wbox[0][threadIdx.x];
        for (int w = 1; w < K1_WAVES; w++) v = threadIdx.x < 3 ? fminf(v, L.wbox[w][threadIdx.x]) : fmaxf(v, L.wbox[w][threadIdx.x]);
        W.bboxes[(size_t)blockIdx.x * 6 + threadIdx.x] = v;
    }
    tmn0 = L.tmin[0]; tmn1 = L.tmin[1]; tmn2 = L.tmin[2];
    const bool any_points = tmn0 <= L.tmax[0];
    uint32_t wg_err = L.err;
    if (any_points) {
        const long long span0 = (long long)L.tmax[0] - tmn0, span1 = (long long)L.tmax[1] - tmn1, span2 = (long long)L.tmax[2] - tmn2;
        if (span0 >= KEY_SPAN_X - 1 || span1 >= KEY_SPAN_Y - 1 || span2 >= KEY_SPAN_Z - 1) wg_err |= ERR_FAST_PATH;
        const int big = 1 << 28;
        if (tmn0 < -big || tmn1 < -big || tmn2 < -big || L.tmax[0] > big || L.tmax[1] > big || L.tmax[2] > big) wg_err |= ERR_RANGE;
    }
    if (wg_err) {
        if (threadIdx.x == 0) atomicOr(&W.ctrl[C_ERR], wg_err);
        return 2;
    }
    return any_points ? 1 : 0;
}

template <int MODE>
__device__ __forceinline__ void fast_flush_records(FastTable &L, const FastParams &P, const VoxWork &W, const int tmn0, const int tmn1, const int tmn2) {
    constexpr int UU = 2;
    const int lane = threadIdx.x & 63;
    const uint32_t key_base = (uint32_t)((((tmn2 << 10) + tmn1) << 10) + tmn0);
    uint32_t bad = 0;
    constexpr int PER_THREAD = (LTAB + K1_THREADS - 1) / K1_THREADS;
    unsigned long long kk[PER_THREAD];
#pragma unroll
    for (int q = 0; q < PER_THREAD; q++) {
        const int e = (int)threadIdx.x + q * K1_THREADS;
        kk[q] = e < LTAB ? L.key[e] : KEY64_EMPTY;
    }
#pragma unroll
    for (int q = 0; q < PER_THREAD; q++) {
        const int e = (int)threadIdx.x + q * K1_THREADS;
        const unsigned long long k64 = kk[q];
        const bool in_use = k64 != KEY64_EMPTY;
        const uint32_t dk = (uint32_t)k64 - key_base, side = (uint32_t)(k64 >> 32);
        const int t[3] = {tmn0 + (int)(dk & 1023u), tmn1 + (int)((dk >> 10) & 1023u), tmn2 + (int)(dk >> 20)};
        const int ib[3] = {P.ib0, P.ib1, P.ib2}, fb[3] = {P.fb0, P.fb1, P.fb2};
        int leaf[3], cell[3];
        bool ok = true;
#pragma unroll
        for (int a = 0; a < 3; a++) {
            if (MODE == 0) {
                leaf[a] = (t[a] - ib[a]) >> 6;
            } else {
                const int *TF = reinterpret_cast<const int *>(&L.faces[FT_TF + a * FACES]);
                int j = ((t[a] - ib[a] - 1) >> 6) - fb[a];
                j = max(1, min(j, FACES - 3));
                const int fm = TF[j - 1], f0 = TF[j], f1 = TF[j + 1], f2 = TF[j + 2];
                const int d = t[a] <= f0 ? -1 : (t[a] > f1 ? 1 : 0);
                const int flo = d < 0 ? fm : d > 0 ? f1 : f0, fhi = d < 0 ? f0 : d > 0 ? f2 : f1;
                j += d;
                ok &= flo < t[a] && t[a] <= fhi;
                leaf[a] = fb[a] + j + (int)((side >> a) & 1u);
            }
            cell[a] = t[a] - ib[a] - 64 * leaf[a] + 2;
            ok &= (unsigned)cell[a] < (unsigned)GRID_DIM;
            ok &= leaf[a] > -(1 << 20) && leaf[a] < (1 << 20);
        }
        uint32_t rec = 0xffffffffu;
        if (in_use) {
            if (ok) {
                const uint32_t ls = fast_leaf_slot(L, pack_leaf(leaf[0], leaf[1], leaf[2]));
                if (ls != 0xffffffffu) rec = (ls << CELL_BITS) | (uint32_t)((cell[2] * GRID_DIM + cell[1]) * GRID_DIM + cell[0]);
                else bad |= ERR_FAST_PATH;
            } else {
                bad |= ERR_CELL_RANGE;
            }
        }
        const unsigned long long vote = __ballot(in_use);
        uint32_t base = 0;
        if (lane == 0 && vote != 0ull) base = atomicAdd(&L.nused, (uint32_t)__popcll(vote));
        base = (uint32_t)__builtin_amdgcn_readfirstlane((int)base);
        if (in_use) {
            const uint32_t at = base + __builtin_amdgcn_mbcnt_hi((uint32_t)(vote >> 32), __builtin_amdgcn_mbcnt_lo((uint32_t)vote, 0u));
            L.used[at] = (uint32_t)e;
            L.rec[at] = rec;
        }
    }
    if (__ballot(bad != 0u) != 0ull) {
        for (int sft = 32; sft > 0; sft >>= 1) bad |= (uint32_t)__shfl_xor((int)bad, sft, 64);
        if (lane == 0) atomicOr(&W.ctrl[C_ERR], bad);
    }
    __syncthreads();
    FAST_STAMP(5);
    const uint32_t nused = L.nused;
#ifdef CWIPC_DEBUG_KNOBS
    if (P.dbg & 512u) return;
#endif
    if (threadIdx.x < LOCAL_LEAVES) {
        const unsigned long long lk = L.leaf_tab[threadIdx.x];
#ifdef CWIPC_DEBUG_KNOBS
        if (P.dbg & 256u) { if (lk != 0ull) L.leaf_gid[threadIdx.x] = threadIdx.x; } else
#endif
        if (lk != 0ull && L.leaf_gid[threadIdx.x] == 0xffffffffu) L.leaf_gid[threadIdx.x] = leaf_lookup_cached(W, P.leaf_mask, lk);
    }
    __syncthreads();
    FAST_STAMP(6);
#ifdef CWIPC_DEBUG_KNOBS
    if (P.dbg & 128u) return;
#endif
    uint32_t okey[PER_THREAD], oold[PER_THREAD];
#pragma unroll
    for (int q = 0; q < PER_THREAD; q++) {
        const uint32_t i = threadIdx.x + (uint32_t)q * K1_THREADS;
        okey[q] = 0xffffffffu; oold[q] = 0xffffffffu;
        if (i >= nused) continue;
        const uint32_t ks = L.rec[i];
        if (ks == 0xffffffffu) continue;
        const uint32_t gid = L.leaf_gid[ks >> CELL_BITS];
        if (gid == 0xffffffffu) continue;
        const uint32_t cell = ks & ((1u << CELL_BITS) - 1);
        okey[q] = (gid << CELL_BITS) | cell;
#ifdef CWIPC_DEBUG_KNOBS
        if (P.dbg & 32u) oold[q] = 0; else
#endif
        oold[q] = atomicOr(&W.bitmaps[(size_t)gid * BITWORDS + (cell >> 5)], 1u << (cell & 31u));
    }
    {
        const int sub = lane & 7;
        const int f1 = sub == 0 ? 0 : sub == 1 ? 1 : sub == 2 ? 2 : sub == 3 ? 3 : 2;
        const int f2 = sub == 0 ? 0 : sub == 1 ? 1 : sub == 2 ? 2 : 3;
        const uint32_t s1 = sub == 3 ? 16u : sub == 4 ? 40u : 0u, s2 = sub == 3 ? 0u : sub == 4 ? 40u : 32u;
        const uint32_t m1 = (sub == 3 || sub == 4) ? 0xffffffu : 0xffffffffu;
        const uint32_t m2 = sub == 2 ? 0xffu : sub == 3 ? 0xffffu : sub == 4 ? 0xffffffu : 0xffffffffu;
        const bool tile_word = sub == 5 || sub == 6;
        const unsigned long long *const w1p = f1 == 0 ? L.a : f1 == 1 ? L.b : f1 == 2 ? L.c : L.d, *const w2p = f2 == 0 ? L.a : f2 == 1 ? L.b : f2 == 2 ? L.c : L.d;
        for (uint32_t i0 = threadIdx.x >> 3; i0 < nused; i0 += UU * (K1_THREADS / 8)) {
            uint32_t e[UU], ks[UU];
#pragma unroll
            for (int u = 0; u < UU; u++) {
                const uint32_t i = i0 + (uint32_t)u * (K1_THREADS / 8);
                e[u] = L.used[i < nused ? i : i0];
                ks[u] = i < nused ? L.rec[i] : 0xffffffffu;
            }
            uint32_t gid[UU], tl[UU];
            unsigned long long w1[UU], w2[UU];
#pragma unroll
            for (int u = 0; u < UU; u++) {
                gid[u] = L.leaf_gid[ks[u] != 0xffffffffu ? ks[u] >> CELL_BITS : 0u];
                if (ks[u] == 0xffffffffu) gid[u] = 0xffffffffu;
                w1[u] = w1p[e[u]]; w2[u] = w2p[e[u]];
                tl[u] = L.tile[e[u]] >> (sub == 6 ? 4 : 0);
            }
#pragma unroll
            for (int u = 0; u < UU; u++) {
                if (gid[u] == 0xffffffffu) continue;
                uint32_t vlo = (uint32_t)(w1[u] >> s1) & m1, vhi = (uint32_t)(w2[u] >> s2) & m2;
                if (tile_word) {
                    vlo = (tl[u] & 1u) | ((tl[u] & 2u) << 15);
                    vhi = ((tl[u] >> 2) & 1u) | ((tl[u] & 8u) << 13);
                }
#ifdef CWIPC_DEBUG_KNOBS
                if (!(P.dbg & 16u))
#endif
                if (sub < 7 && (vlo | vhi) != 0u) atomicAdd(&record_ptr(W, (gid[u] << CELL_BITS) | (ks[u] & ((1u << CELL_BITS) - 1)))[sub], u64_of(vlo, vhi));
            }
        }
    }
#pragma unroll
    for (int q = 0; q < PER_THREAD; q++) {
        const uint32_t k = okey[q];
        const bool fresh = k != 0xffffffffu && !(oold[q] & (1u << (k & 31u)));
        const unsigned long long fv = __ballot(fresh);
        if (fv == 0ull) continue;
        uint32_t base = 0;
        if (lane == 0) base = atomicAdd(&L.nfresh, (uint32_t)__popcll(fv));
        base = (uint32_t)__builtin_amdgcn_readfirstlane((int)base);
        if (fresh) {
            if (P.want_list) L.fresh[base + __builtin_amdgcn_mbcnt_hi((uint32_t)(fv >> 32), __builtin_amdgcn_mbcnt_lo((uint32_t)fv, 0u))] = k;
            const uint32_t sl = slice_of(k);
            uint32_t hs = (sl * 0x9E3779B1u) >> 24;
            bool counted = false;
            for (int probe = 0; probe < 8 && !counted; probe++) {
                const uint32_t tag = atomicCAS(&L.htag[hs], 0u, sl + 1u);
                if (tag == 0u || tag == sl + 1u) {
                    atomicAdd(&L.hcnt[hs], 1u);
                    counted = true;
                }
                hs = (hs + 1) & (HIST - 1);
            }
            if (!counted) atomicAdd(&W.seg_count[sl], 1u);
        }
    }
    __syncthreads();
    FAST_STAMP(7);
    if (threadIdx.x < HIST && L.htag[threadIdx.x]) atomicAdd(&W.seg_count[L.htag[threadIdx.x] - 1u], L.hcnt[threadIdx.x]);
    const uint32_t nfresh = L.nfresh;
    if (threadIdx.x == 0) atomicMax(&W.ctrl[C_MAXLOAD], nused);
    if (!P.want_list) {
        if (threadIdx.x == 0 && nfresh) atomicAdd(&W.ctrl[C_COUNT], nfresh);
        return;
    }
    if (threadIdx.x == 0 && nfresh) L.fresh_base = atomicAdd(&W.ctrl[C_COUNT], nfresh);
    __syncthreads();
    FAST_STAMP(8);
    for (uint32_t i = threadIdx.x; i < nfresh; i += K1_THREADS) {
        const uint32_t idx = L.fresh_base + i;
        if (idx < P.list_cap) W.occupied[idx] = L.fresh[i];
        else atomicOr(&W.ctrl[C_ERR], ERR_LIST_FULL);
    }
}

template <int MODE>
__device__ __forceinline__ void fast_finish(FastTable &L, const FastParams &P, const VoxWork &W, uint32_t err, float bn0, float bn1, float bn2, float bx0, float bx1,
                                            float bx2) {
    int tmn0, tmn1, tmn2;
    if (fast_finish_head(L, P, W, err, bn0, bn1, bn2, bx0, bx1, bx2, tmn0, tmn1, tmn2) != 1) return;
    fast_flush_records<MODE>(L, P, W, tmn0, tmn1, tmn2);
}

template <int MODE>
__global__ void __launch_bounds__(K1_THREADS, 4) voxel_accumulate_fast_kernel(FastParams P, const float *__restrict__ x, const float *__restrict__ y,
                                                                             const float *__restrict__ z, const uint32_t *__restrict__ rgbt, VoxWork W) {
    extern __shared__ __align__(16) unsigned char k1_smem[];
    FastTable &L = *reinterpret_cast<FastTable *>(k1_smem);
    FAST_STAMP(0);

    const int lane = threadIdx.x & 63;
    const int wave = threadIdx.x >> 6;
    uint32_t chunk_lo = blockIdx.x * P.per_wg, chunk_hi = min(chunk_lo + P.per_wg, P.n);
    if (P.range_base_q != 0u) {
        chunk_lo = min(range_first_step(blockIdx.x, P.range_base_q, P.range_inc_q) * (uint32_t)WAVE_STEP, P.n);
        chunk_hi = min(range_first_step(blockIdx.x + 1u, P.range_base_q, P.range_inc_q) * (uint32_t)WAVE_STEP, P.n);
    }
    const int chunk_pts = chunk_lo < chunk_hi ? (int)(chunk_hi - chunk_lo) : 0;
    const int nsteps = (chunk_pts + WAVE_STEP - 1) / WAVE_STEP;
    auto load_step = [&](int step, float4 &ax, float4 &ay, float4 &az, uint4 &aw) __attribute__((always_inline)) {
        const size_t at = (size_t)chunk_lo + (size_t)(uint32_t)__builtin_amdgcn_readfirstlane(step) * WAVE_STEP;
        ax = reinterpret_cast<const float4 *>(x + at)[lane];
        ay = reinterpret_cast<const float4 *>(y + at)[lane];
        az = reinterpret_cast<const float4 *>(z + at)[lane];
        aw = reinterpret_cast<const uint4 *>(rgbt + at)[lane];
    };
    float4 cx = make_float4(0, 0, 0, 0), cy = cx, cz = cx;
    uint4 cw = make_uint4(0, 0, 0, 0);
    int cur = wave < nsteps ? wave : -1;
#ifdef CWIPC_DEBUG_KNOBS
    const int streamers = (P.dbg & 0x20000u) ? 8 : (P.dbg & 0x10000u) ? 12 : K1_WAVES;
    if (wave >= streamers) cur = -1;
#else
    constexpr int streamers = K1_WAVES;
#endif
    if (cur >= 0) load_step(cur, cx, cy, cz, cw);

    constexpr int FT_PER_LANE = (FACE_TABLE_WORDS + K1_THREADS - 1) / K1_THREADS;
    uint32_t ftw[FT_PER_LANE];
    if (MODE == 1) {
        const uint32_t *ft = reinterpret_cast<const uint32_t *>(W.faces);
#pragma unroll
        for (int q = 0; q < FT_PER_LANE; q++) ftw[q] = (int)threadIdx.x + q * K1_THREADS < FACE_TABLE_WORDS ? ft[threadIdx.x + q * K1_THREADS] : 0u;
    }
    auto clear_table = [&]() __attribute__((always_inline)) {
        for (int i = threadIdx.x; i < LTAB; i += K1_THREADS) {
            L.key[i] = KEY64_EMPTY; L.tile[i] = 0;
            L.a[i] = 0; L.b[i] = 0; L.c[i] = 0; L.d[i] = 0;
        }
        if (threadIdx.x < HIST) { L.htag[threadIdx.x] = 0; L.hcnt[threadIdx.x] = 0; }
        if (threadIdx.x == 0) { L.nfresh = 0; L.nused = 0; }
    };
    clear_table();
    if (MODE == 1) {
#pragma unroll
        for (int q = 0; q < FT_PER_LANE; q++)
            if ((int)threadIdx.x + q * K1_THREADS < FACE_TABLE_WORDS) L.faces[threadIdx.x + q * K1_THREADS] = ftw[q];
    }
    if (threadIdx.x < LOCAL_LEAVES) { L.leaf_tab[threadIdx.x] = 0ull; L.leaf_gid[threadIdx.x] = 0xffffffffu; }
    if (threadIdx.x < 3) { L.tmin[threadIdx.x] = INT32_MAX; L.tmax[threadIdx.x] = INT32_MIN; }
    if (threadIdx.x < K1_WAVES * 12) (&L.slab[0][0])[threadIdx.x] = INFINITY;
    if (threadIdx.x < K1_WAVES * 4) (&L.slab_j[0][0])[threadIdx.x] = -1;
    if (threadIdx.x == 0) { L.err = 0; L.next_step = (uint32_t)streamers; }
    __syncthreads();
    FAST_STAMP(1);
    if (wave == K1_WAVES - 1 && lane == 0 && chunk_pts > 0 && nsteps < K1_WAVES)
        fast_scout<MODE>(&L, P.inv_leaf, P.ib0, P.ib1, P.ib2, P.fb0, P.fb1, P.fb2, P.leaf_mask, W.hash_keys, W.hash_ids, W.leaf_keys, W.ctrl, x[chunk_lo], y[chunk_lo], z[chunk_lo]);

    const float inv = P.inv_leaf;
    const f32x2 inv2 = {inv, inv};
    const f32x2 one2 = {1.0f, 1.0f};
    float bn0 = FLT_MAX, bn1 = FLT_MAX, bn2 = FLT_MAX, bx0 = -FLT_MAX, bx1 = -FLT_MAX, bx2 = -FLT_MAX;
    uint32_t err = 0;
    auto step = [&](auto masked_tag, const float4 cx, const float4 cy, const float4 cz, const uint4 cw, int left) __attribute__((always_inline)) {
        constexpr bool MASKED = decltype(masked_tag)::value;
        bool v0 = true, v1 = true, v2 = true, v3 = true;
        if (MASKED) {
            v0 = left > 0 && __builtin_isfinite(cx.x + cy.x + cz.x);
            v1 = left > 1 && __builtin_isfinite(cx.y + cy.y + cz.y);
            v2 = left > 2 && __builtin_isfinite(cx.z + cy.z + cz.z);
            v3 = left > 3 && __builtin_isfinite(cx.w + cy.w + cz.w);
        }
        float mn0, mn1, mn2, mx0, mx1, mx2;
        if (!MASKED) {
            mn0 = min3f(cx.x, cx.y, min2f(cx.z, cx.w)); mx0 = max3f(cx.x, cx.y, max2f(cx.z, cx.w));
            mn1 = min3f(cy.x, cy.y, min2f(cy.z, cy.w)); mx1 = max3f(cy.x, cy.y, max2f(cy.z, cy.w));
            mn2 = min3f(cz.x, cz.y, min2f(cz.z, cz.w)); mx2 = max3f(cz.x, cz.y, max2f(cz.z, cz.w));
        } else {
            const float pinf = INFINITY, ninf = -INFINITY;
            auto lo4 = [&](float a, float b, float c, float d) { return fminf(fminf(v0 ? a : pinf, v1 ? b : pinf), fminf(v2 ? c : pinf, v3 ? d : pinf)); };
            auto hi4 = [&](float a, float b, float c, float d) { return fmaxf(fmaxf(v0 ? a : ninf, v1 ? b : ninf), fmaxf(v2 ? c : ninf, v3 ? d : ninf)); };
            mn0 = lo4(cx.x, cx.y, cx.z, cx.w); mx0 = hi4(cx.x, cx.y, cx.z, cx.w);
            mn1 = lo4(cy.x, cy.y, cy.z, cy.w); mx1 = hi4(cy.x, cy.y, cy.z, cy.w);
            mn2 = lo4(cz.x, cz.y, cz.z, cz.w); mx2 = hi4(cz.x, cz.y, cz.z, cz.w);
        }
        asm("v_min3_f32 %0, %0, %1, %1" : "+v"(bn0) : "v"(mn0)); asm("v_max3_f32 %0, %0, %1, %1" : "+v"(bx0) : "v"(mx0));
        asm("v_min3_f32 %0, %0, %1, %1" : "+v"(bn1) : "v"(mn1)); asm("v_max3_f32 %0, %0, %1, %1" : "+v"(bx1) : "v"(mx1));
        asm("v_min3_f32 %0, %0, %1, %1" : "+v"(bn2) : "v"(mn2)); asm("v_max3_f32 %0, %0, %1, %1" : "+v"(bx2) : "v"(mx2));

#ifdef CWIPC_DEBUG_KNOBS
        if (P.dbg & 4u) { bn0 = fminf(bn0, __uint_as_float(cw.x ^ cw.y ^ cw.z ^ cw.w)); return; }
#endif
        uint32_t h0 = 0, h1 = 0, h2 = 0, h3 = 0;
        bool sided = false;
        bool dead = false;
        float4 sl0, sl1, sl2;
        if (MODE == 1) {
            const float4 *sl = reinterpret_cast<const float4 *>(&L.slab[wave][0]);
            sl0 = sl[0]; sl1 = sl[1]; sl2 = sl[2];
            const bool inside = (mn0 >= sl0.x) & (mx0 < sl0.w) & (mn1 >= sl1.x) & (mx1 < sl1.w) & (mn2 >= sl2.x) & (mx2 < sl2.w);
            if (__builtin_expect(__ballot(!inside) != 0ull, 0)) {
                if (!fast_refit(&L, wave, mn0, mn1, mn2, mx0, mx1, mx2, inv, P.ib0, P.ib1, P.ib2, P.fb0, P.fb1, P.fb2)) { err |= ERR_FAST_PATH; dead = true; }
                sl0 = sl[0]; sl1 = sl[1]; sl2 = sl[2];
            }
            const bool t0 = (mx0 >= sl0.y) & (mn0 < sl0.z), t1 = (mx1 >= sl1.y) & (mn1 < sl1.z), t2 = (mx2 >= sl2.y) & (mn2 < sl2.z);
            if (__builtin_expect(__ballot(t0 | t1 | t2) != 0ull, 0)) {
                sided = true;
                if (__ballot(t0) != 0ull) {
                    h0 |= (cx.x >= sl0.y && cx.x < sl0.z) ? 1u : 0u; h1 |= (cx.y >= sl0.y && cx.y < sl0.z) ? 1u : 0u;
                    h2 |= (cx.z >= sl0.y && cx.z < sl0.z) ? 1u : 0u; h3 |= (cx.w >= sl0.y && cx.w < sl0.z) ? 1u : 0u;
                }
                if (__ballot(t1) != 0ull) {
                    h0 |= (cy.x >= sl1.y && cy.x < sl1.z) ? 2u : 0u; h1 |= (cy.y >= sl1.y && cy.y < sl1.z) ? 2u : 0u;
                    h2 |= (cy.z >= sl1.y && cy.z < sl1.z) ? 2u : 0u; h3 |= (cy.w >= sl1.y && cy.w < sl1.z) ? 2u : 0u;
                }
                if (__ballot(t2) != 0ull) {
                    h0 |= (cz.x >= sl2.y && cz.x < sl2.z) ? 4u : 0u; h1 |= (cz.y >= sl2.y && cz.y < sl2.z) ? 4u : 0u;
                    h2 |= (cz.z >= sl2.y && cz.z < sl2.z) ? 4u : 0u; h3 |= (cz.w >= sl2.y && cz.w < sl2.z) ? 4u : 0u;
                }
            }
        }

        uint32_t k0, k1, k2, k3;
        uint32_t rx0, rx1, rx2, rx3, ry0, ry1, ry2, ry3, rz0, rz1, rz2, rz3;
        {
            const f32x2 qx01 = f32x2{cx.x, cx.y} * inv2, qx23 = f32x2{cx.z, cx.w} * inv2;
            const f32x2 qy01 = f32x2{cy.x, cy.y} * inv2, qy23 = f32x2{cy.z, cy.w} * inv2;
            const f32x2 qz01 = f32x2{cz.x, cz.y} * inv2, qz23 = f32x2{cz.z, cz.w} * inv2;
            const int ix0 = cvt_floor_i32(qx01.x), ix1 = cvt_floor_i32(qx01.y), ix2 = cvt_floor_i32(qx23.x), ix3 = cvt_floor_i32(qx23.y);
            const int iy0 = cvt_floor_i32(qy01.x), iy1 = cvt_floor_i32(qy01.y), iy2 = cvt_floor_i32(qy23.x), iy3 = cvt_floor_i32(qy23.y);
            const int iz0 = cvt_floor_i32(qz01.x), iz1 = cvt_floor_i32(qz01.y), iz2 = cvt_floor_i32(qz23.x), iz3 = cvt_floor_i32(qz23.y);
            k0 = linear_key(ix0, iy0, iz0); k1 = linear_key(ix1, iy1, iz1);
            k2 = linear_key(ix2, iy2, iz2); k3 = linear_key(ix3, iy3, iz3);
            const f32x2 fx01 = f32x2{voxel_fract(qx01.x), voxel_fract(qx01.y)} + one2, fx23 = f32x2{voxel_fract(qx23.x), voxel_fract(qx23.y)} + one2;
            const f32x2 fy01 = f32x2{voxel_fract(qy01.x), voxel_fract(qy01.y)} + one2, fy23 = f32x2{voxel_fract(qy23.x), voxel_fract(qy23.y)} + one2;
            const f32x2 fz01 = f32x2{voxel_fract(qz01.x), voxel_fract(qz01.y)} + one2, fz23 = f32x2{voxel_fract(qz23.x), voxel_fract(qz23.y)} + one2;
            rx0 = __float_as_uint(fx01.x); rx1 = __float_as_uint(fx01.y); rx2 = __float_as_uint(fx23.x); rx3 = __float_as_uint(fx23.y);
            ry0 = __float_as_uint(fy01.x); ry1 = __float_as_uint(fy01.y); ry2 = __float_as_uint(fy23.x); ry3 = __float_as_uint(fy23.y);
            rz0 = __float_as_uint(fz01.x); rz1 = __float_as_uint(fz01.y); rz2 = __float_as_uint(fz23.x); rz3 = __float_as_uint(fz23.y);
        }
        PointAdd a0 = point_add(cw.x), a1 = point_add(cw.y), a2 = point_add(cw.z), a3 = point_add(cw.w);
        const uint32_t tile_u = (uint32_t)__builtin_amdgcn_readfirstlane((int)a0.tile);
        const uint32_t tiles4 = __builtin_amdgcn_perm(__builtin_amdgcn_perm(cw.w, cw.z, 0x0c0c0703u), __builtin_amdgcn_perm(cw.y, cw.x, 0x0c0c0703u), 0x05040100u);
        const bool one_tile = !MASKED && __ballot(tiles4 != tile_u * 0x01010101u) == 0ull;
        if (MASKED) {
            const uint32_t kv = v0 ? k0 : v1 ? k1 : v2 ? k2 : k3, hv = v0 ? h0 : v1 ? h1 : v2 ? h2 : h3;
            k0 = v0 ? k0 : kv; k1 = v1 ? k1 : k0; k2 = v2 ? k2 : k1; k3 = v3 ? k3 : k2;
            h0 = v0 ? h0 : hv; h1 = v1 ? h1 : h0; h2 = v2 ? h2 : h1; h3 = v3 ? h3 : h2;
            auto drop = [](bool v, uint32_t &rx, uint32_t &ry, uint32_t &rz, PointAdd &a) {
                if (!v) { rx = ry = rz = Q_ONE_BITS; a.cr = 0; a.gb = 0; }
            };
            drop(v0, rx0, ry0, rz0, a0); drop(v1, rx1, ry1, rz1, a1); drop(v2, rx2, ry2, rz2, a2); drop(v3, rx3, ry3, rz3, a3);
        }
        const uint32_t C1 = a0.cr, C2 = C1 + a1.cr, C3 = C2 + a2.cr, C4 = C3 + a3.cr;
        const uint32_t G1 = a0.gb, G2 = G1 + a1.gb, G3 = G2 + a2.gb, G4 = G3 + a3.gb;
        uint32_t u0 = tiles4 & 0xffu, u1 = (tiles4 >> 8) & 0xffu, u2 = (tiles4 >> 16) & 0xffu, u3 = tiles4 >> 24;
        if (MASKED) {
            const uint32_t uv = v0 ? u0 : v1 ? u1 : v2 ? u2 : u3;
            u0 = v0 ? u0 : uv; u1 = v1 ? u1 : u0; u2 = v2 ? u2 : u1; u3 = v3 ? u3 : u2;
        }
        const uint32_t tiles = u0 | (u1 << 8) | (u2 << 16) | (u3 << 24);
        const uint32_t hp = h0 | (h1 << 3) | (h2 << 6) | (h3 << 9);

        const uint32_t X1 = rx0 + Q_NEG_ONE_BITS, X2 = X1 + rx1 + Q_NEG_ONE_BITS, X3 = X2 + rx2 + Q_NEG_ONE_BITS, X4 = X3 + rx3 + Q_NEG_ONE_BITS;
        const uint32_t Y1 = ry0 + Q_NEG_ONE_BITS, Y2 = Y1 + ry1 + Q_NEG_ONE_BITS, Y3 = Y2 + ry2 + Q_NEG_ONE_BITS, Y4 = Y3 + ry3 + Q_NEG_ONE_BITS;
        const uint32_t Z1 = rz0 + Q_NEG_ONE_BITS, Z2 = Z1 + rz1 + Q_NEG_ONE_BITS, Z3 = Z2 + rz2 + Q_NEG_ONE_BITS, Z4 = Z3 + rz3 + Q_NEG_ONE_BITS;

#ifdef CWIPC_DEBUG_KNOBS
        if (P.dbg & 2u) { bx0 = fmaxf(bx0, __uint_as_float((X4 ^ Y4 ^ Z4 ^ C4 ^ G4 ^ k0 ^ k1 ^ k2 ^ k3 ^ hp ^ tiles) & 0x3fffffffu)); return; }
#endif
        const uint32_t kn = (uint32_t)__builtin_amdgcn_update_dpp(0, (int)k0, 0x130, 0xf, 0xf, true);
        bool b1 = k1 != k0, b2 = k2 != k1, b3 = k3 != k2, b4 = (k3 != kn) | (lane == 63);
        if (__builtin_expect(sided, 0)) {
            const uint32_t hn = (uint32_t)__builtin_amdgcn_update_dpp(0, (int)hp, 0x130, 0xf, 0xf, true) & 7u;
            const uint32_t hx = hp ^ (hp >> 3);
            b1 |= (hx & 7u) != 0u; b2 |= (hx & 0x38u) != 0u; b3 |= (hx & 0x1c0u) != 0u; b4 |= (hp >> 9) != hn;
        }
        if (__builtin_expect(!one_tile, 0)) {
            const uint32_t un = (uint32_t)__builtin_amdgcn_update_dpp(0, (int)tiles, 0x130, 0xf, 0xf, true) & 0xffu;
            const uint32_t tx = tiles ^ (tiles >> 8);
            b1 |= (tx & 0xffu) != 0u; b2 |= (tx & 0xff00u) != 0u; b3 |= (tx & 0xff0000u) != 0u; b4 |= (tiles >> 24) != un;
        }
        const uint32_t bits = (b1 ? 1u : 0u) | (b2 ? 2u : 0u) | (b3 ? 4u : 0u) | (b4 ? 8u : 0u);
        const unsigned long long has = __ballot(bits != 0u);
        const uint32_t lt_lo = lane >= 32 ? 0xffffffffu : (1u << lane) - 1u, lt_hi = lane > 32 ? (1u << (lane - 32)) - 1u : 0u;
        const uint32_t below_lo = (uint32_t)has & lt_lo, below_hi = (uint32_t)(has >> 32) & lt_hi;
        const bool none_below = (below_lo | below_hi) == 0u;
        const int prev_lane = below_hi ? 63 - __clz((int)below_hi) : 31 - __clz((int)below_lo);
        const int paddr = prev_lane << 2;
        auto tile_at = [&](uint32_t j) { return one_tile ? tile_u : ((tiles >> (8u * j)) & 0xffu); };
        auto side_at = [&](uint32_t j) { return sided ? ((hp >> (3u * j)) & 7u) : 0u; };
        auto field = [&](uint32_t A1, uint32_t A2, uint32_t A3, uint32_t A4) {
            const uint32_t E = wave_inclusive_scan(A4) - A4;
            const uint32_t Lf = E + (b4 ? A4 : b3 ? A3 : b2 ? A2 : A1);
            const uint32_t got = (uint32_t)__builtin_amdgcn_ds_bpermute(paddr, (int)Lf);
            const uint32_t first = b1 ? A1 : b2 ? A2 : b3 ? A3 : A4;
            return E + first - (none_below ? 0u : got);
        };
#ifdef CWIPC_DEBUG_KNOBS
        if (P.dbg & 1u) {
            const uint32_t t = field(C1, C2, C3, C4) ^ field(X1, X2, X3, X4) ^ field(Y1, Y2, Y3, Y4) ^ field(Z1, Z2, Z3, Z4) ^ field(G1, G2, G3, G4);
            bx1 = fmaxf(bx1, __uint_as_float(t & 0x3fffffffu));
            return;
        }
#endif
        if (!dead) {
            const uint32_t j0 = b1 ? 0u : b2 ? 1u : b3 ? 2u : 3u;
            const uint32_t key0 = b1 ? k0 : b2 ? k1 : b3 ? k2 : k3, side0 = side_at(j0);
            uint32_t slot;
            unsigned long long found = KEY64_EMPTY;
            if (!MASKED) found = fast_find_begin(L, key0, side0, bits != 0u, slot);
            const uint32_t cnt0 = field(C1, C2, C3, C4);
            const uint32_t sx0 = field(X1, X2, X3, X4);
            const uint32_t sy0 = field(Y1, Y2, Y3, Y4);
            __builtin_amdgcn_sched_barrier(0);
            const bool act0 = bits != 0u && (!MASKED || (cnt0 >> 16) != 0u);
            if (MASKED) found = fast_find_begin(L, key0, side0, act0, slot);
            const bool ok0 = fast_find_end(L, key0, side0, act0, found, slot, err);
            if (ok0) {
                atomicAdd(&L.a[slot], u64_of(sx0, 0u));
                atomicAdd(&L.b[slot], u64_of(sy0, 0u));
            }
            const uint32_t sz0 = field(Z1, Z2, Z3, Z4);
            const uint32_t sg0 = field(G1, G2, G3, G4);
            __builtin_amdgcn_sched_barrier(0);
            fast_add_rest(L, slot, ok0, sz0, cnt0, sg0, tile_at(j0));
            uint32_t left_bits = bits & (bits - 1u);
            if (__builtin_expect(__ballot(left_bits != 0u) != 0ull, 0)) {
                uint32_t BX = b1 ? X1 : b2 ? X2 : X3, BY = b1 ? Y1 : b2 ? Y2 : Y3, BZ = b1 ? Z1 : b2 ? Z2 : Z3, BC = b1 ? C1 : b2 ? C2 : C3, BG = b1 ? G1 : b2 ? G2 : G3;
#pragma unroll 1
                for (int round = 1; round < 4; round++) {
                    const bool mine = left_bits != 0u;
                    const bool at2 = (left_bits & 2u) != 0u, at3 = !at2 && (left_bits & 4u) != 0u;
                    const uint32_t TX = at2 ? X2 : at3 ? X3 : X4, TY = at2 ? Y2 : at3 ? Y3 : Y4, TZ = at2 ? Z2 : at3 ? Z3 : Z4;
                    const uint32_t TC = at2 ? C2 : at3 ? C3 : C4, TG = at2 ? G2 : at3 ? G3 : G4;
                    const uint32_t j = at2 ? 1u : at3 ? 2u : 3u;
                    const uint32_t cnt = TC - BC;
                    const bool ok = fast_find(L, at2 ? k1 : at3 ? k2 : k3, side_at(j), mine && (!MASKED || (cnt >> 16) != 0u), slot, err);
                    if (ok) {
                        atomicAdd(&L.a[slot], u64_of(TX - BX, 0u));
                        atomicAdd(&L.b[slot], u64_of(TY - BY, 0u));
                    }
                    fast_add_rest(L, slot, ok, TZ - BZ, cnt, TG - BG, tile_at(j));
                    BX = TX; BY = TY; BZ = TZ; BC = TC; BG = TG;
                    left_bits &= left_bits - 1u;
                    if (__ballot(left_bits != 0u) == 0ull) break;
                }
            }
        }
    };

    auto grab = [&]() -> int {
        uint32_t t = 0;
        if (lane == 0) t = atomicAdd(&L.next_step, 1u);
        t = (uint32_t)__builtin_amdgcn_readfirstlane((int)t);
        return t < (uint32_t)nsteps ? (int)t : -1;
    };
    int nxt = cur >= 0 ? grab() : -1;
#pragma unroll 1
    while (cur >= 0) {
        cur = __builtin_amdgcn_readfirstlane(cur);
        nxt = __builtin_amdgcn_readfirstlane(nxt);
        float4 nx = cx, ny = cy, nz = cz;
        uint4 nw = cw;
        if (nxt >= 0) load_step(nxt, nx, ny, nz, nw);
        const int left = chunk_pts - cur * WAVE_STEP - lane * 4;
        const f32x2 sx = f32x2{cx.x, cx.y} + f32x2{cx.z, cx.w}, sy = f32x2{cy.x, cy.y} + f32x2{cy.z, cy.w}, sz = f32x2{cz.x, cz.y} + f32x2{cz.z, cz.w};
        const f32x2 sa = (sx + sy) + sz;
        const bool odd = left < 4 || !__builtin_isfinite(sa.x + sa.y);
        if (__builtin_expect(__ballot(odd) == 0ull, 1)) step(std::false_type{}, cx, cy, cz, cw, left);
        else step(std::true_type{}, cx, cy, cz, cw, left);
        cx = nx; cy = ny; cz = nz; cw = nw;
        cur = nxt;
        if (cur >= 0) nxt = grab();
    }

    FAST_STAMP(2);
#ifdef CWIPC_DEBUG_KNOBS
    if (blockIdx.x == 0 && lane == 0 && wave < K1_WAVES) g_fast_wave_done[wave] = wall_clock64();
#endif
    fast_finish<MODE>(L, P, W, err, bn0, bn1, bn2, bx0, bx1, bx2);
}
```

Measured before the change: 234,400 Mpoints/s.

## Run two smaller fast-accumulate workgroups per CU with halved LDS hash table

Reshapes the fast voxel accumulate kernel to 640-thread workgroups with a 1024-entry LDS hash table, so that two workgroups can share one CU's LDS, and sizes the grid and workspace for two workgroups per CU. To save registers, per-thread bounding boxes move into an LDS array that is unioned with the finish-phase scratch and updated with LDS atomic min/max. Loads now use a scalar base address, the previous-lane mask is computed with a 64-bit shift and clz, and the tail iteration leaves the next-step registers undefined instead of copying them. The risks are more hash-table overflow and fallback from the smaller table, plus extra LDS atomic traffic for the bounding-box updates.

```diff
diff --git a/cwipc_util_amd/csrc/kernels_voxel.hip b/cwipc_util_amd/csrc/kernels_voxel.hip
--- a/cwipc_util_amd/csrc/kernels_voxel.hip
+++ b/cwipc_util_amd/csrc/kernels_voxel.hip
@@ -560,7 +560,7 @@
 }
 
 bool VoxCall::setup_pass() {
-    if (!ensure_workspace(ws, n, leaf_cap, (uint32_t)nwaves, c.stream)) return false;
+    if (!ensure_workspace(ws, n, leaf_cap, std::max((uint32_t)nwaves, (uint32_t)cus * FAST_WGS_PER_CU), c.stream)) return false;
     P.leaf_mask = 4 * ws.leaf_cap - 1;
     P.list_cap = (uint32_t)(ws.list_cap > 0xffffffffu ? 0xffffffffu : ws.list_cap);
     seq = ++ws.seq ? ws.seq : ++ws.seq;
@@ -648,10 +648,10 @@
         F.dbg = fast_dbg;
 #endif
         if (mode == 0) {
-            CW_LAUNCH("voxel_accumulate", voxel_accumulate_fast_kernel<0>, dim3(fplan.blocks), dim3(K1_THREADS), sizeof(FastTable), c.stream, F, src.x(),
+            CW_LAUNCH("voxel_accumulate", voxel_accumulate_fast_kernel<0>, dim3(fplan.blocks), dim3(FAST_THREADS), sizeof(FastTable), c.stream, F, src.x(),
                       src.y(), src.z(), src.rgbt(), W);
         } else {
-            CW_LAUNCH("voxel_accumulate", voxel_accumulate_fast_kernel<1>, dim3(fplan.blocks), dim3(K1_THREADS), sizeof(FastTable), c.stream, F, src.x(),
+            CW_LAUNCH("voxel_accumulate", voxel_accumulate_fast_kernel<1>, dim3(fplan.blocks), dim3(FAST_THREADS), sizeof(FastTable), c.stream, F, src.x(),
                       src.y(), src.z(), src.rgbt(), W);
         }
     } else if (mode == 0) {
@@ -784,10 +784,10 @@
                 }
             }
         }
-        unsigned long long wd[K1_WAVES];
+        unsigned long long wd[FAST_WAVES];
         if (hipMemcpyFromSymbol(wd, HIP_SYMBOL(g_fast_wave_done), sizeof(wd)) == hipSuccess) {
             std::string line = "debug: workgroup 0, waves done with their steps at (us):";
-            for (int w = 0; w < K1_WAVES; w++) line += " " + std::to_string((double)(wd[w] - st[0][0]) * 0.01).substr(0, 5);
+            for (int w = 0; w < FAST_WAVES; w++) line += " " + std::to_string((double)(wd[w] - st[0][0]) * 0.01).substr(0, 5);
             cwipc_log(CWIPC_LOG_LEVEL_WARNING, "cwipc_downsample", line);
         }
     }
diff --git a/cwipc_util_amd/csrc/voxel_anchor.hpp b/cwipc_util_amd/csrc/voxel_anchor.hpp
--- a/cwipc_util_amd/csrc/voxel_anchor.hpp
+++ b/cwipc_util_amd/csrc/voxel_anchor.hpp
@@ -103,12 +103,13 @@
 struct FastPlan { uint32_t blocks, per_wg, base_q, inc_q; };
 inline FastPlan fast_plan(size_t n, int cus, int stagger_knob) {
     const size_t steps_total = (n + WAVE_STEP - 1) / WAVE_STEP;
-    const size_t wg_steps = std::min<size_t>(std::max<size_t>((steps_total + cus - 1) / cus, 1), MAX_POINTS_PER_WAVE * K1_WAVES / WAVE_STEP);
+    const size_t slots = (size_t)(cus > 0 ? cus : 1) * FAST_WGS_PER_CU;
+    const size_t wg_steps = std::min<size_t>(std::max<size_t>((steps_total + slots - 1) / slots, 1), FAST_MAX_WG_STEPS);
     FastPlan plan{(uint32_t)((steps_total + wg_steps - 1) / wg_steps), (uint32_t)(wg_steps * WAVE_STEP), 0u, 0u};
     const uint32_t fast_blocks = plan.blocks;
     if (stagger_knob > 0 && stagger_knob < 60 && fast_blocks >= 64 && steps_total >= (size_t)24 * fast_blocks && n < ((size_t)1 << 31)) {
         const double mean_q = (double)steps_total * 1024.0 / (double)fast_blocks, s_frac = stagger_knob / 100.0;
-        const size_t max_steps = MAX_POINTS_PER_WAVE * K1_WAVES / WAVE_STEP;
+        const size_t max_steps = FAST_MAX_WG_STEPS;
         uint32_t inc = (uint32_t)ceil(2.0 * s_frac * mean_q / (double)(fast_blocks - 1));
         uint32_t base = (uint32_t)ceil(mean_q * (1.0 - s_frac));
         while (range_first_step(fast_blocks, base, inc) < steps_total) base++;
diff --git a/cwipc_util_amd/csrc/voxel_common.hpp b/cwipc_util_amd/csrc/voxel_common.hpp
--- a/cwipc_util_amd/csrc/voxel_common.hpp
+++ b/cwipc_util_amd/csrc/voxel_common.hpp
@@ -15,6 +15,12 @@
 constexpr size_t MAX_POINTS_PER_WAVE = 3840;
 constexpr int LTAB = 2048;
 constexpr int LTAB_PROBES = 32;
+constexpr int FAST_THREADS = 640;
+constexpr int FAST_WAVES = FAST_THREADS / 64;
+constexpr int FAST_LTAB = 1024;
+constexpr int FAST_LTAB_BITS = 10;
+constexpr int FAST_WGS_PER_CU = 2;
+constexpr size_t FAST_MAX_WG_STEPS = 240;
 constexpr int GRID_DIM = 68;
 constexpr int CELLS = GRID_DIM * GRID_DIM * GRID_DIM;
 constexpr int CELL_BITS = 19;
diff --git a/cwipc_util_amd/csrc/voxel_k1_fast.inc b/cwipc_util_amd/csrc/voxel_k1_fast.inc
--- a/cwipc_util_amd/csrc/voxel_k1_fast.inc
+++ b/cwipc_util_amd/csrc/voxel_k1_fast.inc
@@ -1,7 +1,7 @@
 
 #ifdef CWIPC_DEBUG_KNOBS
 __device__ unsigned long long g_fast_stamps[2][16];
-__device__ unsigned long long g_fast_wave_done[K1_WAVES];
+__device__ unsigned long long g_fast_wave_done[FAST_WAVES];
 __device__ unsigned long long g_wg_times[1024][4];
 #define FAST_STAMP(i) do { if (threadIdx.x == 0) { const unsigned long long t_ = wall_clock64(); if (blockIdx.x == 0 || blockIdx.x == gridDim.x / 2) g_fast_stamps[blockIdx.x ? 1 : 0][i] = t_; \
     if (blockIdx.x < 1024 && ((i) == 0 || (i) == 2 || (i) == 3 || (i) == 7)) g_wg_times[blockIdx.x][(i) == 0 ? 0 : (i) == 2 ? 1 : (i) == 3 ? 2 : 3] = t_; } } while (0)
@@ -26,26 +26,32 @@
 };
 
 struct FastTable {
-    unsigned long long key[LTAB];
-    uint32_t tile[LTAB];
-    unsigned long long a[LTAB];
-    unsigned long long b[LTAB];
-    unsigned long long c[LTAB];
-    unsigned long long d[LTAB];
+    unsigned long long key[FAST_LTAB];
+    uint32_t tile[FAST_LTAB];
+    unsigned long long a[FAST_LTAB];
+    unsigned long long b[FAST_LTAB];
+    unsigned long long c[FAST_LTAB];
+    unsigned long long d[FAST_LTAB];
     uint32_t faces[FACE_TABLE_WORDS];
     uint32_t htag[HIST], hcnt[HIST];
     unsigned long long leaf_tab[LOCAL_LEAVES];
     uint32_t leaf_gid[LOCAL_LEAVES];
-    alignas(16) float slab[K1_WAVES][12];
-    int slab_j[K1_WAVES][4];
+    alignas(16) float slab[FAST_WAVES][12];
+    int slab_j[FAST_WAVES][4];
     int tmin[3], tmax[3];
     uint32_t nfresh, fresh_base, nused, err;
     uint32_t next_step;
-    float wbox[K1_WAVES][6];
-    alignas(16) uint32_t used[LTAB];
-    uint32_t rec[LTAB];
-    uint32_t fresh[LTAB];
+    float wbox[FAST_WAVES][6];
+    union {
+        struct {
+            alignas(16) uint32_t used[FAST_LTAB];
+            uint32_t rec[FAST_LTAB];
+            uint32_t fresh[FAST_LTAB];
+        };
+        float box[6][FAST_THREADS];
+    };
 };
+static_assert(FAST_WGS_PER_CU * ((sizeof(FastTable) + 2047) / 2048 * 2048) <= 160 * 1024, "two fast workgroups must share a CU's LDS");
 
 __device__ __forceinline__ uint32_t linear_key(int ix, int iy, int iz) {
     uint32_t t, k;
@@ -64,6 +70,16 @@
     return r;
 }
 
+typedef uint32_t u32x4 __attribute__((ext_vector_type(4)));
+template <class T>
+__device__ __forceinline__ u32x4 load16_scalar_base(const T *p, int lane) {
+    uint32_t lo = (uint32_t)__builtin_amdgcn_readfirstlane((int)(uint32_t)reinterpret_cast<uintptr_t>(p));
+    uint32_t hi = (uint32_t)__builtin_amdgcn_readfirstlane((int)(uint32_t)(reinterpret_cast<uintptr_t>(p) >> 32));
+    asm("" : "+s"(lo), "+s"(hi));
+    typedef const u32x4 __attribute__((address_space(1))) *global_ptr;
+    return reinterpret_cast<global_ptr>(((uintptr_t)hi << 32) | lo)[lane];
+}
+
 __device__ __forceinline__ int cvt_floor_i32(float v) {
     int r;
     asm("v_cvt_flr_i32_f32 %0, %1" : "=v"(r) : "v"(v));
@@ -71,9 +87,9 @@
 }
 
 __device__ __forceinline__ uint32_t fast_hash(uint32_t key, uint32_t side) {
-    static_assert(LTAB <= 2048 && (LTAB & (LTAB - 1)) == 0, "11 bits at most");
+    static_assert(FAST_LTAB == (1 << FAST_LTAB_BITS) && FAST_LTAB_BITS <= 11, "11 bits at most");
     const uint32_t t = key ^ (key >> 13) ^ (side << 7);
-    return (__umul24(t, 0x9E3779u) >> 13) & (uint32_t)(LTAB - 1);
+    return (__umul24(t, 0x9E3779u) >> (24 - FAST_LTAB_BITS)) & (uint32_t)(FAST_LTAB - 1);
 }
 
 __device__ __forceinline__ unsigned long long fast_find_begin(FastTable &L, uint32_t key, uint32_t side, bool active, uint32_t &slot) {
@@ -89,7 +105,7 @@
     for (int probe = 1; probe < LTAB_PROBES; probe++) {
         if (__ballot(pending) == 0ull) break;
         if (pending) {
-            slot = (slot + 1) & (LTAB - 1);
+            slot = (slot + 1) & (FAST_LTAB - 1);
             old = atomicCAS(&L.key[slot], KEY64_EMPTY, key64);
             if (old == KEY64_EMPTY || old == key64) pending = false;
         }
@@ -246,7 +262,7 @@
     FAST_STAMP(3);
     if (threadIdx.x < 6) {
         float v = L.wbox[0][threadIdx.x];
-        for (int w = 1; w < K1_WAVES; w++) v = threadIdx.x < 3 ? fminf(v, L.wbox[w][threadIdx.x]) : fmaxf(v, L.wbox[w][threadIdx.x]);
+        for (int w = 1; w < FAST_WAVES; w++) v = threadIdx.x < 3 ? fminf(v, L.wbox[w][threadIdx.x]) : fmaxf(v, L.wbox[w][threadIdx.x]);
         W.bboxes[(size_t)blockIdx.x * 6 + threadIdx.x] = v;
     }
     tmn0 = L.tmin[0]; tmn1 = L.tmin[1]; tmn2 = L.tmin[2];
@@ -271,16 +287,16 @@
     const int lane = threadIdx.x & 63;
     const uint32_t key_base = (uint32_t)((((tmn2 << 10) + tmn1) << 10) + tmn0);
     uint32_t bad = 0;
-    constexpr int PER_THREAD = (LTAB + K1_THREADS - 1) / K1_THREADS;
+    constexpr int PER_THREAD = (FAST_LTAB + FAST_THREADS - 1) / FAST_THREADS;
     unsigned long long kk[PER_THREAD];
 #pragma unroll
     for (int q = 0; q < PER_THREAD; q++) {
-        const int e = (int)threadIdx.x + q * K1_THREADS;
-        kk[q] = e < LTAB ? L.key[e] : KEY64_EMPTY;
+        const int e = (int)threadIdx.x + q * FAST_THREADS;
+        kk[q] = e < FAST_LTAB ? L.key[e] : KEY64_EMPTY;
     }
 #pragma unroll
     for (int q = 0; q < PER_THREAD; q++) {
-        const int e = (int)threadIdx.x + q * K1_THREADS;
+        const int e = (int)threadIdx.x + q * FAST_THREADS;
         const unsigned long long k64 = kk[q];
         const bool in_use = k64 != KEY64_EMPTY;
         const uint32_t dk = (uint32_t)k64 - key_base, side = (uint32_t)(k64 >> 32);
@@ -352,7 +368,7 @@
     uint32_t okey[PER_THREAD], oold[PER_THREAD];
 #pragma unroll
     for (int q = 0; q < PER_THREAD; q++) {
-        const uint32_t i = threadIdx.x + (uint32_t)q * K1_THREADS;
+        const uint32_t i = threadIdx.x + (uint32_t)q * FAST_THREADS;
         okey[q] = 0xffffffffu; oold[q] = 0xffffffffu;
         if (i >= nused) continue;
         const uint32_t ks = L.rec[i];
@@ -375,11 +391,11 @@
         const uint32_t m2 = sub == 2 ? 0xffu : sub == 3 ? 0xffffu : sub == 4 ? 0xffffffu : 0xffffffffu;
         const bool tile_word = sub == 5 || sub == 6;
         const unsigned long long *const w1p = f1 == 0 ? L.a : f1 == 1 ? L.b : f1 == 2 ? L.c : L.d, *const w2p = f2 == 0 ? L.a : f2 == 1 ? L.b : f2 == 2 ? L.c : L.d;
-        for (uint32_t i0 = threadIdx.x >> 3; i0 < nused; i0 += UU * (K1_THREADS / 8)) {
+        for (uint32_t i0 = threadIdx.x >> 3; i0 < nused; i0 += UU * (FAST_THREADS / 8)) {
             uint32_t e[UU], ks[UU];
 #pragma unroll
             for (int u = 0; u < UU; u++) {
-                const uint32_t i = i0 + (uint32_t)u * (K1_THREADS / 8);
+                const uint32_t i = i0 + (uint32_t)u * (FAST_THREADS / 8);
                 e[u] = L.used[i < nused ? i : i0];
                 ks[u] = i < nused ? L.rec[i] : 0xffffffffu;
             }
@@ -444,7 +460,7 @@
     if (threadIdx.x == 0 && nfresh) L.fresh_base = atomicAdd(&W.ctrl[C_COUNT], nfresh);
     __syncthreads();
     FAST_STAMP(8);
-    for (uint32_t i = threadIdx.x; i < nfresh; i += K1_THREADS) {
+    for (uint32_t i = threadIdx.x; i < nfresh; i += FAST_THREADS) {
         const uint32_t idx = L.fresh_base + i;
         if (idx < P.list_cap) W.occupied[idx] = L.fresh[i];
         else atomicOr(&W.ctrl[C_ERR], ERR_LIST_FULL);
@@ -460,14 +476,14 @@
 }
 
 template <int MODE>
-__global__ void __launch_bounds__(K1_THREADS, 4) voxel_accumulate_fast_kernel(FastParams P, const float *__restrict__ x, const float *__restrict__ y,
+__global__ void __launch_bounds__(FAST_THREADS, 5) voxel_accumulate_fast_kernel(FastParams P, const float *__restrict__ x, const float *__restrict__ y,
                                                                              const float *__restrict__ z, const uint32_t *__restrict__ rgbt, VoxWork W) {
     extern __shared__ __align__(16) unsigned char k1_smem[];
     FastTable &L = *reinterpret_cast<FastTable *>(k1_smem);
     FAST_STAMP(0);
 
     const int lane = threadIdx.x & 63;
-    const int wave = threadIdx.x >> 6;
+    const int wave = __builtin_amdgcn_readfirstlane((int)(threadIdx.x >> 6));
     uint32_t chunk_lo = blockIdx.x * P.per_wg, chunk_hi = min(chunk_lo + P.per_wg, P.n);
     if (P.range_base_q != 0u) {
         chunk_lo = min(range_first_step(blockIdx.x, P.range_base_q, P.range_inc_q) * (uint32_t)WAVE_STEP, P.n);
@@ -477,31 +493,33 @@
     const int nsteps = (chunk_pts + WAVE_STEP - 1) / WAVE_STEP;
     auto load_step = [&](int step, float4 &ax, float4 &ay, float4 &az, uint4 &aw) __attribute__((always_inline)) {
         const size_t at = (size_t)chunk_lo + (size_t)(uint32_t)__builtin_amdgcn_readfirstlane(step) * WAVE_STEP;
-        ax = reinterpret_cast<const float4 *>(x + at)[lane];
-        ay = reinterpret_cast<const float4 *>(y + at)[lane];
-        az = reinterpret_cast<const float4 *>(z + at)[lane];
-        aw = reinterpret_cast<const uint4 *>(rgbt + at)[lane];
+        const u32x4 rx = load16_scalar_base(x + at, lane), ry = load16_scalar_base(y + at, lane), rz = load16_scalar_base(z + at, lane);
+        const u32x4 rw = load16_scalar_base(rgbt + at, lane);
+        ax = make_float4(__uint_as_float(rx.x), __uint_as_float(rx.y), __uint_as_float(rx.z), __uint_as_float(rx.w));
+        ay = make_float4(__uint_as_float(ry.x), __uint_as_float(ry.y), __uint_as_float(ry.z), __uint_as_float(ry.w));
+        az = make_float4(__uint_as_float(rz.x), __uint_as_float(rz.y), __uint_as_float(rz.z), __uint_as_float(rz.w));
+        aw = make_uint4(rw.x, rw.y, rw.z, rw.w);
     };
     float4 cx = make_float4(0, 0, 0, 0), cy = cx, cz = cx;
     uint4 cw = make_uint4(0, 0, 0, 0);
     int cur = wave < nsteps ? wave : -1;
 #ifdef CWIPC_DEBUG_KNOBS
-    const int streamers = (P.dbg & 0x20000u) ? 8 : (P.dbg & 0x10000u) ? 12 : K1_WAVES;
+    const int streamers = (P.dbg & 0x20000u) ? 5 : (P.dbg & 0x10000u) ? 8 : FAST_WAVES;
     if (wave >= streamers) cur = -1;
 #else
-    constexpr int streamers = K1_WAVES;
+    constexpr int streamers = FAST_WAVES;
 #endif
     if (cur >= 0) load_step(cur, cx, cy, cz, cw);
 
-    constexpr int FT_PER_LANE = (FACE_TABLE_WORDS + K1_THREADS - 1) / K1_THREADS;
+    constexpr int FT_PER_LANE = (FACE_TABLE_WORDS + FAST_THREADS - 1) / FAST_THREADS;
     uint32_t ftw[FT_PER_LANE];
     if (MODE == 1) {
         const uint32_t *ft = reinterpret_cast<const uint32_t *>(W.faces);
 #pragma unroll
-        for (int q = 0; q < FT_PER_LANE; q++) ftw[q] = (int)threadIdx.x + q * K1_THREADS < FACE_TABLE_WORDS ? ft[threadIdx.x + q * K1_THREADS] : 0u;
+        for (int q = 0; q < FT_PER_LANE; q++) ftw[q] = (int)threadIdx.x + q * FAST_THREADS < FACE_TABLE_WORDS ? ft[threadIdx.x + q * FAST_THREADS] : 0u;
     }
     auto clear_table = [&]() __attribute__((always_inline)) {
-        for (int i = threadIdx.x; i < LTAB; i += K1_THREADS) {
+        for (int i = threadIdx.x; i < FAST_LTAB; i += FAST_THREADS) {
             L.key[i] = KEY64_EMPTY; L.tile[i] = 0;
             L.a[i] = 0; L.b[i] = 0; L.c[i] = 0; L.d[i] = 0;
         }
@@ -512,23 +530,26 @@
     if (MODE == 1) {
 #pragma unroll
         for (int q = 0; q < FT_PER_LANE; q++)
-            if ((int)threadIdx.x + q * K1_THREADS < FACE_TABLE_WORDS) L.faces[threadIdx.x + q * K1_THREADS] = ftw[q];
+            if ((int)threadIdx.x + q * FAST_THREADS < FACE_TABLE_WORDS) L.faces[threadIdx.x + q * FAST_THREADS] = ftw[q];
     }
     if (threadIdx.x < LOCAL_LEAVES) { L.leaf_tab[threadIdx.x] = 0ull; L.leaf_gid[threadIdx.x] = 0xffffffffu; }
     if (threadIdx.x < 3) { L.tmin[threadIdx.x] = INT32_MAX; L.tmax[threadIdx.x] = INT32_MIN; }
-    if (threadIdx.x < K1_WAVES * 12) (&L.slab[0][0])[threadIdx.x] = INFINITY;
-    if (threadIdx.x < K1_WAVES * 4) (&L.slab_j[0][0])[threadIdx.x] = -1;
+    if (threadIdx.x < FAST_WAVES * 12) (&L.slab[0][0])[threadIdx.x] = INFINITY;
+    if (threadIdx.x < FAST_WAVES * 4) (&L.slab_j[0][0])[threadIdx.x] = -1;
     if (threadIdx.x == 0) { L.err = 0; L.next_step = (uint32_t)streamers; }
+#pragma unroll
+    for (int i = 0; i < 6; i++) L.box[i][threadIdx.x] = i < 3 ? FLT_MAX : -FLT_MAX;
     __syncthreads();
     FAST_STAMP(1);
-    if (wave == K1_WAVES - 1 && lane == 0 && chunk_pts > 0 && nsteps < K1_WAVES)
+    if (wave == FAST_WAVES - 1 && lane == 0 && chunk_pts > 0 && nsteps < FAST_WAVES)
         fast_scout<MODE>(&L, P.inv_leaf, P.ib0, P.ib1, P.ib2, P.fb0, P.fb1, P.fb2, P.leaf_mask, W.hash_keys, W.hash_ids, W.leaf_keys, W.ctrl, x[chunk_lo], y[chunk_lo], z[chunk_lo]);
 
     const float inv = P.inv_leaf;
     const f32x2 inv2 = {inv, inv};
     const f32x2 one2 = {1.0f, 1.0f};
-    float bn0 = FLT_MAX, bn1 = FLT_MAX, bn2 = FLT_MAX, bx0 = -FLT_MAX, bx1 = -FLT_MAX, bx2 = -FLT_MAX;
     uint32_t err = 0;
+    auto box_min = [&](int i, float v) __attribute__((always_inline)) { (void)__hip_atomic_fetch_min(&L.box[i][threadIdx.x], v, __ATOMIC_RELAXED, __HIP_MEMORY_SCOPE_WORKGROUP); };
+    auto box_max = [&](int i, float v) __attribute__((always_inline)) { (void)__hip_atomic_fetch_max(&L.box[i][threadIdx.x], v, __ATOMIC_RELAXED, __HIP_MEMORY_SCOPE_WORKGROUP); };
     auto step = [&](auto masked_tag, const float4 cx, const float4 cy, const float4 cz, const uint4 cw, int left) __attribute__((always_inline)) {
         constexpr bool MASKED = decltype(masked_tag)::value;
         bool v0 = true, v1 = true, v2 = true, v3 = true;
@@ -551,12 +572,12 @@
             mn1 = lo4(cy.x, cy.y, cy.z, cy.w); mx1 = hi4(cy.x, cy.y, cy.z, cy.w);
             mn2 = lo4(cz.x, cz.y, cz.z, cz.w); mx2 = hi4(cz.x, cz.y, cz.z, cz.w);
         }
-        asm("v_min3_f32 %0, %0, %1, %1" : "+v"(bn0) : "v"(mn0)); asm("v_max3_f32 %0, %0, %1, %1" : "+v"(bx0) : "v"(mx0));
-        asm("v_min3_f32 %0, %0, %1, %1" : "+v"(bn1) : "v"(mn1)); asm("v_max3_f32 %0, %0, %1, %1" : "+v"(bx1) : "v"(mx1));
-        asm("v_min3_f32 %0, %0, %1, %1" : "+v"(bn2) : "v"(mn2)); asm("v_max3_f32 %0, %0, %1, %1" : "+v"(bx2) : "v"(mx2));
-
-#ifdef CWIPC_DEBUG_KNOBS
-        if (P.dbg & 4u) { bn0 = fminf(bn0, __uint_as_float(cw.x ^ cw.y ^ cw.z ^ cw.w)); return; }
+        box_min(0, mn0); box_max(3, mx0);
+        box_min(1, mn1); box_max(4, mx1);
+        box_min(2, mn2); box_max(5, mx2);
+
+#ifdef CWIPC_DEBUG_KNOBS
+        if (P.dbg & 4u) { box_min(0, __uint_as_float((cw.x ^ cw.y ^ cw.z ^ cw.w) & 0x3fffffffu)); return; }
 #endif
         uint32_t h0 = 0, h1 = 0, h2 = 0, h3 = 0;
         bool sided = false;
@@ -634,7 +655,7 @@
         const uint32_t Z1 = rz0 + Q_NEG_ONE_BITS, Z2 = Z1 + rz1 + Q_NEG_ONE_BITS, Z3 = Z2 + rz2 + Q_NEG_ONE_BITS, Z4 = Z3 + rz3 + Q_NEG_ONE_BITS;
 
 #ifdef CWIPC_DEBUG_KNOBS
-        if (P.dbg & 2u) { bx0 = fmaxf(bx0, __uint_as_float((X4 ^ Y4 ^ Z4 ^ C4 ^ G4 ^ k0 ^ k1 ^ k2 ^ k3 ^ hp ^ tiles) & 0x3fffffffu)); return; }
+        if (P.dbg & 2u) { box_max(3, __uint_as_float((X4 ^ Y4 ^ Z4 ^ C4 ^ G4 ^ k0 ^ k1 ^ k2 ^ k3 ^ hp ^ tiles) & 0x3fffffffu)); return; }
 #endif
         const uint32_t kn = (uint32_t)__builtin_amdgcn_update_dpp(0, (int)k0, 0x130, 0xf, 0xf, true);
         bool b1 = k1 != k0, b2 = k2 != k1, b3 = k3 != k2, b4 = (k3 != kn) | (lane == 63);
@@ -650,10 +671,9 @@
         }
         const uint32_t bits = (b1 ? 1u : 0u) | (b2 ? 2u : 0u) | (b3 ? 4u : 0u) | (b4 ? 8u : 0u);
         const unsigned long long has = __ballot(bits != 0u);
-        const uint32_t lt_lo = lane >= 32 ? 0xffffffffu : (1u << lane) - 1u, lt_hi = lane > 32 ? (1u << (lane - 32)) - 1u : 0u;
-        const uint32_t below_lo = (uint32_t)has & lt_lo, below_hi = (uint32_t)(has >> 32) & lt_hi;
-        const bool none_below = (below_lo | below_hi) == 0u;
-        const int prev_lane = below_hi ? 63 - __clz((int)below_hi) : 31 - __clz((int)below_lo);
+        const unsigned long long below = (has << (63 - lane)) & 0x7fffffffffffffffull;
+        const bool none_below = below == 0ull;
+        const int prev_lane = lane - __clzll((long long)below);
         const int paddr = prev_lane << 2;
         auto tile_at = [&](uint32_t j) { return one_tile ? tile_u : ((tiles >> (8u * j)) & 0xffu); };
         auto side_at = [&](uint32_t j) { return sided ? ((hp >> (3u * j)) & 7u) : 0u; };
@@ -667,7 +687,7 @@
 #ifdef CWIPC_DEBUG_KNOBS
         if (P.dbg & 1u) {
             const uint32_t t = field(C1, C2, C3, C4) ^ field(X1, X2, X3, X4) ^ field(Y1, Y2, Y3, Y4) ^ field(Z1, Z2, Z3, Z4) ^ field(G1, G2, G3, G4);
-            bx1 = fmaxf(bx1, __uint_as_float(t & 0x3fffffffu));
+            box_max(4, __uint_as_float(t & 0x3fffffffu));
             return;
         }
 #endif
@@ -728,9 +748,18 @@
     while (cur >= 0) {
         cur = __builtin_amdgcn_readfirstlane(cur);
         nxt = __builtin_amdgcn_readfirstlane(nxt);
-        float4 nx = cx, ny = cy, nz = cz;
-        uint4 nw = cw;
-        if (nxt >= 0) load_step(nxt, nx, ny, nz, nw);
+        float4 nx, ny, nz;
+        uint4 nw;
+        if (nxt >= 0) {
+            load_step(nxt, nx, ny, nz, nw);
+        } else {
+            unsigned long long u0, u1, u2, u3, u4, u5, u6, u7;
+            asm("" : "=v"(u0), "=v"(u1), "=v"(u2), "=v"(u3), "=v"(u4), "=v"(u5), "=v"(u6), "=v"(u7));
+            const auto lo = [](unsigned long long u) { return __uint_as_float((uint32_t)u); };
+            const auto hi = [](unsigned long long u) { return __uint_as_float((uint32_t)(u >> 32)); };
+            nx = make_float4(lo(u0), hi(u0), lo(u1), hi(u1)); ny = make_float4(lo(u2), hi(u2), lo(u3), hi(u3));
+            nz = make_float4(lo(u4), hi(u4), lo(u5), hi(u5)); nw = make_uint4((uint32_t)u6, (uint32_t)(u6 >> 32), (uint32_t)u7, (uint32_t)(u7 >> 32));
+        }
         const int left = chunk_pts - cur * WAVE_STEP - lane * 4;
         const f32x2 sx = f32x2{cx.x, cx.y} + f32x2{cx.z, cx.w}, sy = f32x2{cy.x, cy.y} + f32x2{cy.z, cy.w}, sz = f32x2{cz.x, cz.y} + f32x2{cz.z, cz.w};
         const f32x2 sa = (sx + sy) + sz;
@@ -744,7 +773,9 @@
 
     FAST_STAMP(2);
 #ifdef CWIPC_DEBUG_KNOBS
-    if (blockIdx.x == 0 && lane == 0 && wave < K1_WAVES) g_fast_wave_done[wave] = wall_clock64();
-#endif
+    if (blockIdx.x == 0 && lane == 0 && wave < FAST_WAVES) g_fast_wave_done[wave] = wall_clock64();
+#endif
+    const float bn0 = L.box[0][threadIdx.x], bn1 = L.box[1][threadIdx.x], bn2 = L.box[2][threadIdx.x];
+    const float bx0 = L.box[3][threadIdx.x], bx1 = L.box[4][threadIdx.x], bx2 = L.box[5][threadIdx.x];
     fast_finish<MODE>(L, P, W, err, bn0, bn1, bn2, bx0, bx1, bx2);
 }
```

Measured after the change: 177,200 Mpoints/s. 0.756x the previous value.
